# RedhawkSDR/psk_soft

Measured on AMD Instinct MI355X. Metric: complex IQ Msamples/s, QPSK 8 sps, 4096 ch; % HBM roofline at 1/2/4/8 GPUs, higher is better.
Workload: dtype f32

## Files before the change

### psk_soft_amd/csrc/psk_capi.cpp

```cpp
#include <hip/hip_runtime_api.h>
#include <hip/hip_vector_types.h>

#include <atomic>
#include <cmath>
#include <condition_variable>
#include <cstdio>
#include <cstdlib>
#include <cstring>
#include <functional>
#include <mutex>
#include <new>
#include <string>
#include <thread>
#include <vector>

#include "psk_acquire.h"
#include "psk_ctl.h"
#include "psk_gather.h"
#include "psk_plan.h"
#include "psk_quality.h"
#include "psk_soft_hip.h"
#include "psk_tune.h"

namespace psk {
// ... 600 lines not shown
    const psk::ChanCtl &c0 = h->ctl[ch0];
    for (uint32_t i = 1; i < nch; i++)
        if (!ctl_equal(c0, h->ctl[ch0 + i])) {
            h->mixed_lo = ch0, h->mixed_hi = ch0 + nch, h->mixed_ttl = 256;
            return nullptr;
        }
    psk_soft_handle::UniRun *run = nullptr;
    for (int k = psk_soft_handle::kUniRuns - 1; k >= 0; k--)
        run = h->uni[k].hi == h->uni[k].lo ? &h->uni[k] : run;
    if (!run) {
        run = &h->uni[0];
        run_sync(h, *run);
    }
    run->lo = ch0, run->hi = ch0 + nch, run->lazy = false;
    return run;
}
void plan_stamped(Round &r)
{
    psk_soft_handle *const h = r.h;
    if (!h->opt_stamp || r.cont || r.nch < 16u || !(r.run = uniform_run(h, r.ch0, r.nch)))
        return;
    r.stamp_ctl = r.run->lazy ? r.run->ctl : h->ctl[r.ch0];
    psk::ChanPlan &p0 = r.plans[0];
    const psk_soft_packet_t &k0 = r.pkts[0];
    if (psk::plan_call(r.stamp_ctl, r.lim, k0, r.outs[0], p0, false) != PSK_SOFT_OK || p0.mode == psk::PLAN_SKIP || misaligned(r, p0))
        return;
    p0.lf_flags |= r.extra_flags;
    p0.handed_over = r.handed_over;
    account(p0, r.lim, r.res, r.nch);
    const psk_soft_output_t o0 = r.outs[0];
    uint32_t i = 1;
    for (const uint32_t n = r.res.long_call ? 0u : r.nch; i < n; i++) {
        const psk_soft_packet_t &k = r.pkts[i];
        psk_soft_output_t &o = r.outs[i];
        if (k.n_floats != k0.n_floats || k.format != k0.format || k.present != k0.present || k.sri_mode != k0.sri_mode || k.sriChanged != k0.sriChanged ||
            k.inputQueueFlushed != k0.inputQueueFlushed || std::memcmp(&k.sri_xdelta, &k0.sri_xdelta, sizeof(double)) != 0)
            break;
        if (p0.n_out > o.cap_symbols && (o.soft || o.phase))
            break;
        psk::ChanPlan &p = r.plans[i];
        p = p0;
        p.in = k.data, p.soft = o.soft, p.bits = o.bits, p.phase = o.phase, p.sidx = o.sampleIndex;
        if (misaligned(r, p))
            break;
        o.ret = o0.ret, o.n_symbols = o0.n_symbols, o.n_bits = o0.n_bits, o.n_sampleIndex = o0.n_sampleIndex;
        o.sri_pushed = o0.sri_pushed, o.sri_soft_xdelta = o0.sri_soft_xdelta, o.sri_bits_xdelta = o0.sri_bits_xdelta;
        o.n_warn = o0.n_warn;
    }
    r.stamped = i == r.nch;
    if (!r.stamped)
        r.res = PlanSummary();
}
void plan_each(Round &r)
{
    psk::ChanCtl *const next = r.h->ctl_next.data() + r.ch0;
    const psk::ChanCtl *const cur = r.h->ctl.data() + r.ch0;
    PlanSummary &res = r.res;
    for (uint32_t i = 0; i < r.nch; i++) {
        next[i] = cur[i];
        psk::ChanPlan &p = r.plans[i];
        psk_soft_status st = psk::plan_call(next[i], r.lim, r.pkts[i], r.outs[i], p, r.cont && (r.cont[i] & 1u));
        if (st != PSK_SOFT_OK) {
            res.st = st, res.bad = i, res.why = st == PSK_SOFT_ERR_INVALID_ARG ? 3 : 0;
            return;
        }
        if (p.mode == psk::PLAN_SKIP)
            continue;
        if (misaligned(r, p)) {
            res.st = PSK_SOFT_ERR_INVALID_ARG, res.bad = i, res.why = 2;
            return;
        }
        p.lf_flags |= r.extra_flags;
        p.handed_over = r.handed_over;
        if (r.cont && (r.cont[i] & 2u))
            p.lf_flags |= psk::PLAN_NO_WRAP;
        if (r.cont && (r.cont[i] & 4u))
            p.lf_flags |= psk::PLAN_CARRY_DRIFT;
        account(p, r.lim, res, 1u);
    }
}
psk_soft_status refusal(const Round &r)
{
    const PlanSummary &res = r.res;
    if (res.why == 2)
        return fail(PSK_SOFT_ERR_INVALID_ARG,
                    "psk_soft_process: packet data must be 8-byte aligned (CS16: 4) (CS8: 2) (CF16: 4), soft 8, bits 4, phase 4, sampleIndex 4");
    char buf[160];
    if (res.why == 3) {
        std::snprintf(buf, sizeof buf, "psk_soft_process: channel %u: unknown packet format %u (PSK_SOFT_FORMAT_CF32 = 0, CS16 = 1, CS8 = 3, CF16 = 4)",
                      r.ch0 + res.bad, (unsigned)r.pkts[res.bad].format);
        return fail(PSK_SOFT_ERR_INVALID_ARG, buf);
    }
    std::snprintf(buf, sizeof buf, "psk_soft_process: channel %u refused (status %d)", r.ch0 + res.bad, (int)res.st);
    return fail(res.st, buf);
}
void commit(Round &r)
{
    psk_soft_handle *const h = r.h;
    if (r.stamped) {
        r.run->ctl = r.stamp_ctl;
        r.run->mode = r.plans[0].mode;
        r.run->lazy = true;
        return;
    }
    if (r.ch0 == 0 && r.nch == h->nch)
        h->ctl.swap(h->ctl_next);
    else
        std::memcpy(static_cast<void *>(h->ctl.data() + r.ch0), h->ctl_next.data() + r.ch0, sizeof(psk::ChanCtl) * r.nch);
    for (uint32_t i = 0; i < r.nch; i++) h->last_mode[r.ch0 + i] = r.plans[i].mode;
}
psk_soft_status wait_for_overlapping_calls(Round &r)
{
    psk_soft_handle *const h = r.h;
    for (int k = 0; k < kPlanSlots; k++)
        if (k != r.slot && h->ev_used[k] && h->slot_stream[k] != r.stream && h->slot_ch0[k] < r.ch0 + r.nch &&
            r.ch0 < h->slot_ch0[k] + h->slot_nch[k]) {
            PSK_HIP(hipStreamWaitEvent(r.stream, h->ev[k], 0));
            for (int a = 0; a < kAuxStreams; a++)
                if (h->slot_aux_used[k][a])
                    PSK_HIP(hipStreamWaitEvent(r.stream, h->slot_aux_ev[k][a], 0));
        }
    return PSK_SOFT_OK;
}
void move_in_place_back(Round &r)
{
    const psk_soft_handle *const h = r.h;
    if (r.stamped && !(r.plans[0].lf_flags & kInPlaceFlags))
        return;
    for (int S = 2; S <= 16; S++) {
        LaunchSet &fl = r.res.cls[S][1];
        uint32_t cnt = fl.cnt, mb = fl.max_blocks, mn = fl.max_n;
        for (const psk::PktFormat &f : psk::kPktFormats) {
            const LaunchSet &c = r.res.cls[S][f.cls];
            cnt += c.cnt;
            mb = c.max_blocks > mb ? c.max_blocks : mb;
            mn = c.max_n > mn ? c.max_n : mn;
        }
        if (cnt == fl.cnt || !h->opt_tiled || !psk::tile_front_has(S, 1))
            continue;
        const bool pipe = h->opt_pipe == 2 ? mb >= 4u
                                           : h->opt_pipe && h->opt_tiled == 1 && cnt >= kPipeMinChannels && cnt <= kPipeMaxChannels &&
                                                 mb >= kPipeMinBlocks && !r.cont && mn + 128u <= kPipeMaxYLen;
        const bool tiled = h->opt_tiled == 2 || pipe || (cnt <= kTiledFewChannels && mb >= kTiledMinBlocksFew) ||
                           (cnt <= kTiledMaxChannels && mb >= kTiledMinBlocks);
        if (!tiled)
            continue;
        fl.cnt = cnt, fl.max_blocks = mb, fl.max_n = mn;
        for (const psk::PktFormat &f : psk::kPktFormats) {
            LaunchSet &c = r.res.cls[S][f.cls];
            fl.max_A = fl.max_A > c.max_A ? fl.max_A : c.max_A;
            fl.blocks += c.blocks;
            c = LaunchSet{};
        }
        for (uint32_t i = 0; i < r.nch; i++)
            if (r.plans[i].S == (uint32_t)S)
                r.plans[i].lf_flags &= ~kInPlaceFlags;
    }
}
void fill_lists(Round &r)
{
    r.h_list = reinterpret_cast<uint32_t *>(r.h->h_plans[r.slot] + r.nch);
    r.d_plans = r.h->d_plans[r.slot];
    r.d_list = reinterpret_cast<const uint32_t *>(r.d_plans + r.nch);
    uint32_t run = 0;
    each_set(r.res, [&](LaunchSet &s) {
        s.off = run;
        run += s.cnt;
    });
    r.far_rows = r.res.anyf.cnt + r.res.widef.cnt + r.res.quietf.cnt;
    if (r.stamped) {
        for (uint32_t i = 0; i < r.nch; i++) r.h_list[i] = i;
        return;
    }
    for (uint32_t i = 0; i < r.nch; i++)
        if (LaunchSet *const s = set_of(r.plans[i], r.lim, r.res))
            r.h_list[s->off++] = i;
    each_set(r.res, [](LaunchSet &s) { s.off -= s.cnt; });
}
struct TileRule {
    uint64_t k_min;
    uint32_t z;
    bool lengthen;
    bool pfit;
};
void place_tiles(Round &r, LaunchSet &s, const TileRule &rule)
{
    const uint64_t blocks_z = s.blocks * rule.z;
    uint64_t K = blocks_z / kTiledTargetTiles;
    K = K < rule.k_min ? rule.k_min : K > 16 ? 16 : K;
    const uint64_t k_win = (s.max_A + 127u) / 128u;
    if (rule.lengthen && K < k_win) {
        const uint64_t k_fill = blocks_z / (kTiledTargetTiles / 2);
        const uint64_t k_long = k_win > 64 ? 64 : k_win;
        K = k_fill > k_long ? k_long : k_fill > K ? k_fill : K;
    }
    s.tiled = true;
    s.K = (uint8_t)K;
    s.tiles_max = (uint32_t)((s.max_blocks + K - 1) / K);
    for (uint32_t i = 0; i < s.cnt; i++) {
        psk::ChanPlan &p = r.plans[r.h_list[s.off + i]];
        const uint64_t nb = (p.n_out + 127u) / 128u;
        p.lf_flags |= psk::PLAN_TILED;
        if (rule.pfit && r.h->opt_pfit && p.lf_len0 == p.lf_n && p.lf_n >= 2)
            p.lf_flags |= psk::PLAN_PFIT;
        p.tile_blocks = (uint32_t)K;
        p.tile_base = (uint32_t)r.tile_count;
        p.tile_off = r.tile_syms;
        r.tile_count += (size_t)((nb + K - 1) / K);
        r.tile_syms += (size_t)nb * 128u;
    }
}
void place_ranges(Round &r, LaunchSet &s)
{
    s.piped = true;
    const uint32_t T = s.tiles_max;
    uint32_t tr = (uint32_t)(kTiledTargetTiles / s.cnt);
    tr = tr < 1u ? 1u : tr;
    if (r.h->opt_pipe == 2 && tr > 3u)
        tr = 3u;
    if (const char *e = std::getenv("PSK_SOFT_PIPE_RANGE_TILES"))
        tr = std::atoi(e) > 0 ? (uint32_t)std::atoi(e) : tr;
    if ((T + tr - 1) / tr > kPipeMaxRanges)
        tr = (T + kPipeMaxRanges - 1) / kPipeMaxRanges;
    s.pipe_tiles = tr;
    if (s.off + s.cnt > r.pipe_need)
        r.pipe_need = s.off + s.cnt;
}
void place_all(Round &r)
{
    const psk_soft_handle *const h = r.h;
    PlanSummary &res = r.res;
    r.wide_z = (res.wide.cnt || res.widef.cnt) ? psk::wide_chunks(res.wide.max_S > res.widef.max_S ? res.wide.max_S : res.widef.max_S) : 0u;
    if (res.wide.cnt)
        place_tiles(r, res.wide, TileRule{1, r.wide_z, true, true});
    if (res.widef.cnt)
        place_tiles(r, res.widef, TileRule{1, r.wide_z, true, false});
    r.wide_rec_need = r.tile_syms * r.wide_z * psk::wide_rec_bytes(), r.wide_stat_need = r.tile_count * r.wide_z * psk::wide_stat_bytes();
    if (res.any.cnt)
        place_tiles(r, res.any, TileRule{2, 1, true, true});
    if (res.anyf.cnt)
        place_tiles(r, res.anyf, TileRule{2, 1, true, false});
    r.pf_syms = r.tile_syms, r.pf_count = r.tile_count;
    for (int pass = 0; pass < (h->opt_tiled ? 2 : 0); pass++) {
        for (int S : kFastS)
            for (int H : kClassH) {
                LaunchSet &s = res.cls[S][H];
                if (!s.cnt || class_pkt(H) || !psk::tile_front_has(S, class_H(H)))
                    continue;
                const bool pipe = (h->opt_pipe == 2 ? s.max_blocks >= 4u
                                                    : h->opt_pipe && h->opt_tiled == 1 && s.cnt >= kPipeMinChannels && s.cnt <= kPipeMaxChannels &&
                                                          s.max_blocks >= kPipeMinBlocks) &&
                                  !r.cont && s.max_n + 128u <= kPipeMaxYLen && (size_t)s.blocks * 128u <= kPipeMaxSymbols;
                if (pipe != (pass == 1))
                    continue;
                if (!pipe && h->opt_tiled == 1 &&
                    !((s.cnt <= kTiledFewChannels && s.max_blocks >= kTiledMinBlocksFew) || (s.cnt <= kTiledMaxChannels && s.max_blocks >= kTiledMinBlocks)))
                    continue;
                place_tiles(r, s, TileRule{2, 1, false, !pipe});
                if (pipe)
                    place_ranges(r, s);
            }
        if (pass == 0)
            r.pf_syms = r.tile_syms, r.pf_count = r.tile_count;
    }
}

struct ScratchBuf {
    void **buf;
    size_t bytes;
};
template <class T>
inline ScratchBuf scratch_buf(T **p, size_t n) { return ScratchBuf{reinterpret_cast<void **>(p), sizeof(T) * n}; }
inline size_t plus_quarter(size_t need) { return need + need / 4; }
hipError_t grow_scratch(std::initializer_list<ScratchBuf> bufs, bool *got)
{
    if (const hipError_t e = hipDeviceSynchronize())
        return e;
    for (const ScratchBuf &b : bufs) (void)hipFree(*b.buf), *b.buf = nullptr;
    *got = true;
    for (const ScratchBuf &b : bufs) *got = *got && hipMalloc(b.buf, b.bytes) == hipSuccess;
    if (!*got) {
        (void)hipGetLastError();
        for (const ScratchBuf &b : bufs) (void)hipFree(*b.buf), *b.buf = nullptr;
    }
    return hipSuccess;
}
void to_reference_order(psk::ChanPlan &p)
{
    p.mode = p.S == 1u ? psk::PLAN_SEQ_S1 : psk::PLAN_SEQ;
    p.lf_flags &= ~(uint32_t)(psk::PLAN_TILED | psk::PLAN_PFIT | psk::PLAN_ANYFRONT | psk::PLAN_FARFIT);
}
psk_soft_status scratch_tiles(Round &r)
{
    psk_soft_handle *const h = r.h;
    PlanSummary &res = r.res;
    if (!r.tile_syms || (r.tile_syms <= h->tile_sym_cap && r.tile_count <= h->tile_cap && r.pf_syms <= h->pf_sym_cap && r.pf_count <= h->pf_cap))
        return PSK_SOFT_OK;
    h->tile_cap = h->tile_sym_cap = h->pf_cap = h->pf_sym_cap = 0;
    const size_t syms = plus_quarter(r.tile_syms), cnt = plus_quarter(r.tile_count);
    const size_t psyms = plus_quarter(r.pf_syms) + 128u, pcnt = plus_quarter(r.pf_count) + 1u;
    psk::PfScratch &pf = h->pf;
    bool got = false;
    PSK_HIP(grow_scratch({scratch_buf(&h->d_tiles, cnt), scratch_buf(&h->d_traw, syms), scratch_buf(&h->d_test, syms), scratch_buf(&h->d_ts, syms),
                          scratch_buf(&pf.k, psyms), scratch_buf(&pf.y, psyms), scratch_buf(&pf.S, psyms), scratch_buf(&pf.c, psyms),
                          scratch_buf(&pf.tt, psyms), scratch_buf(&pf.xs, psyms), scratch_buf(&pf.tile, pcnt),
                          scratch_buf(&pf.blk, psyms / 128u + 1u), scratch_buf(&pf.walk, psyms / 128u + 1u)},
                         &got));
    if (got && !pf.chan) {
        got = hipMalloc((void **)&pf.chan, sizeof(psk::PfChan) * h->nch) == hipSuccess &&
              hipMemset(pf.chan, 0, sizeof(psk::PfChan) * h->nch) == hipSuccess && hipHostMalloc((void **)&pf.hint, 64) == hipSuccess;
        if (got)
            *pf.hint = 0u;
    }
    if (got) {
        h->tile_cap = cnt, h->tile_sym_cap = syms, h->pf_cap = pcnt, h->pf_sym_cap = psyms;
        return PSK_SOFT_OK;
    }
    (void)hipGetLastError();
    for (uint32_t i = 0; i < r.nch; i++) {
        psk::ChanPlan &p = r.plans[i];
        if (p.lf_flags & psk::PLAN_ANYFRONT) {
            to_reference_order(p);
            res.any_seq = true;
        }
        p.lf_flags &= ~(uint32_t)(psk::PLAN_TILED | psk::PLAN_PFIT);
    }
    res.any.cnt = res.wide.cnt = res.anyf.cnt = res.widef.cnt = 0;
    for (int S : kFastS)
        for (int H : kClassH) res.cls[S][H].tiled = res.cls[S][H].piped = false;
    r.tile_syms = 0;
    return PSK_SOFT_OK;
}
psk_soft_status scratch_wide(Round &r)
{
    psk_soft_handle *const h = r.h;
    PlanSummary &res = r.res;
    if (!(res.wide.cnt || res.widef.cnt) || (r.wide_rec_need <= h->wide_rec_cap && r.wide_stat_need <= h->wide_stat_cap))
        return PSK_SOFT_OK;
    h->wide_rec_cap = h->wide_stat_cap = 0;
    const size_t rb = plus_quarter(r.wide_rec_need), sb = plus_quarter(r.wide_stat_need);
    bool got = false;
    PSK_HIP(grow_scratch({ScratchBuf{&h->d_wide_rec, rb}, ScratchBuf{&h->d_wide_stat, sb}}, &got));
    if (got) {
        h->wide_rec_cap = rb, h->wide_stat_cap = sb;
        return PSK_SOFT_OK;
    }
    for (const LaunchSet *s : {&res.wide, &res.widef})
        for (uint32_t i = 0; i < s->cnt; i++) to_reference_order(r.plans[r.h_list[s->off + i]]);
    res.wide.cnt = res.widef.cnt = 0;
    res.any_seq = true;
    return PSK_SOFT_OK;
}
psk_soft_status scratch_far_rows(Round &r)
{
    psk_soft_handle *const h = r.h;
    PlanSummary &res = r.res;
    if (!r.far_rows)
        return PSK_SOFT_OK;
    const uint32_t *const list = r.h_list + res.anyf.off;
    if (h->far_row.empty())
        h->far_row.assign(h->nch, 0u);
    uint32_t used = h->far_rows_used;
    for (uint32_t i = 0; i < r.far_rows; i++)
        if (!h->far_row[r.ch0 + list[i]])
            used++;
    bool got = true;
    if (used > h->far_rows_cap) {
        h->far_rows_cap = 0;
        const uint32_t cap = plus_quarter(used) < h->nch ? (uint32_t)plus_quarter(used) : h->nch;
        PSK_HIP(grow_scratch({ScratchBuf{(void **)&h->d_far_y, psk::far_ring_bytes() * cap}}, &got));
        if (got)
            h->far_rows_cap = cap;
    }
    for (uint32_t i = 0; i < r.far_rows; i++) {
        psk::ChanPlan &p = r.plans[list[i]];
        if (got) {
            uint32_t &row = h->far_row[r.ch0 + list[i]];
            if (!row)
                row = ++h->far_rows_used;
            p.far_row = row - 1u;
        } else if (p.n_out) {
            to_reference_order(p);
        }
    }
    if (!got) {
        if (res.quietf.cnt)
            return fail(PSK_SOFT_ERR_HIP, "psk_soft_process: out of device memory for the fit window of a far channel (PSK_SOFT_OPT_FAR_FIT)");
        res.anyf.cnt = res.widef.cnt = 0;
        res.any_seq = true;
    }
    return PSK_SOFT_OK;
}
psk_soft_status scratch_wide_seq(Round &r)
{
    psk_soft_handle *const h = r.h;
    for (uint32_t i = 0; i < r.nch; i++)
        if (r.plans[i].mode != psk::PLAN_SKIP && r.plans[i].S > kSeqMaxS) {
            r.n_wide_seq++;
            r.wide_seq_S = r.plans[i].S > r.wide_seq_S ? r.plans[i].S : r.wide_seq_S;
        }
    const size_t need = (size_t)r.n_wide_seq * r.wide_seq_S;
    if (need <= h->wide_symE_cap)
        return PSK_SOFT_OK;
    h->wide_symE_cap = 0;
    bool got = false;
    PSK_HIP(grow_scratch({scratch_buf(&h->d_wide_symE, plus_quarter(need))}, &got));
    if (!got)
        return fail(PSK_SOFT_ERR_HIP, "psk_soft_process: out of device memory for the symbolEnergy rows of wide symbols");
    h->wide_symE_cap = plus_quarter(need);
    return PSK_SOFT_OK;
}
psk_soft_status scratch_order(Round &r)
{
    psk_soft_handle *const h = r.h;
    if (!r.tile_syms && !r.n_wide_seq)
        return PSK_SOFT_OK;
    if (!h->tile_ev)
        PSK_HIP(hipEventCreateWithFlags(&h->tile_ev, hipEventDisableTiming));
    if (r.tile_syms) {
        if (h->pf.hint && *static_cast<volatile uint32_t *>(h->pf.hint)) {
            *static_cast<volatile uint32_t *>(h->pf.hint) = 0u;
            h->pf_second_ttl = 16;
        } else if (h->pf_second_ttl) {
            h->pf_second_ttl--;
        }
        r.pf_second = h->opt_pfit == 2 || h->pf_second_ttl > 0;
    }
    if (h->tile_ev_used && h->tile_stream != r.stream)
        PSK_HIP(hipStreamWaitEvent(r.stream, h->tile_ev, 0));
    if (!r.tile_syms || !r.pipe_need)
        return PSK_SOFT_OK;
    if (r.pipe_need > h->pipe_cap) {
        h->pipe_cap = 0;
        const size_t cap = plus_quarter(r.pipe_need);
        bool got = false;
        PSK_HIP(grow_scratch({ScratchBuf{&h->d_pipe_carry, psk::pipe_carry_bytes() * cap}, scratch_buf(&h->d_pipe_y, kPipeMaxYLen * cap)}, &got));
        if (got)
            h->pipe_cap = cap;
        else
            for (int S : kFastS)
                for (int H : kClassH) r.res.cls[S][H].piped = false;
    }
    if (!h->pipe_st[0]) {
        int prio_lo = 0, prio_hi = 0;
        PSK_HIP(hipDeviceGetStreamPriorityRange(&prio_lo, &prio_hi));
        for (hipStream_t &q : h->pipe_st) PSK_HIP(hipStreamCreateWithPriority(&q, hipStreamNonBlocking, prio_hi));
        for (hipEvent_t &e : h->pipe_ev) PSK_HIP(hipEventCreateWithFlags(&e, hipEventDisableTiming));
    }
    return PSK_SOFT_OK;
}
int cvt_format(const psk::ChanPlan &p)
{
    if (p.mode == psk::PLAN_SKIP || !p.n_in)
        return -1;
    for (int f = 0; f < psk::kNumPktFormats; f++)
        if ((p.lf_flags & psk::kPktFormats[f].flag) && !(p.lf_flags & psk::kPktFormats[f].in_place))
            return f;
    return -1;
}
psk_soft_status conversion_descriptors(Round &r)
{
    psk_soft_handle *const h = r.h;
    size_t need = 0;
    for (uint32_t i = 0; i < r.nch; i++)
        if (const int f = cvt_format(r.plans[i]); f >= 0) {
            need += align_up(sizeof(float2) * r.plans[i].n_in, 128);
            r.n_cvt++, r.n_cvt_f[f]++;
        }
    if (!r.n_cvt)
        return PSK_SOFT_OK;
    CvtScratch *cv = &h->cvt[0], *own = nullptr;
    for (auto &c : h->cvt) {
        cv = c.last_use < cv->last_use ? &c : cv;
        own = !own && c.buf && c.stream == r.stream ? &c : own;
    }
    r.cv = cv = own ? own : cv;
    if (!cv->ev)
        PSK_HIP(hipEventCreateWithFlags(&cv->ev, hipEventDisableTiming));
    if (cv->ev_used && cv->stream != r.stream)
        PSK_HIP(hipStreamWaitEvent(r.stream, cv->ev, 0));
    if (need > cv->cap) {
        cv->cap = 0;
        const size_t cap = align_up(plus_quarter(need), 4096);
        bool got = false;
        PSK_HIP(grow_scratch({ScratchBuf{(void **)&cv->buf, cap}}, &got));
        if (!got)
            return fail(PSK_SOFT_ERR_HIP, "psk_soft_process: out of device memory for the conversion of CS16 / CS8 / CF16 packets");
        cv->cap = cap;
    }
    cv->stream = r.stream, cv->last_use = ++h->cvt_calls;
    psk::CvtDesc *const desc =
        reinterpret_cast<psk::CvtDesc *>(reinterpret_cast<char *>(psk::plan_header(h->h_plans[r.slot])) + slot_cvt_offset(r.nch));
    size_t off = 0;
    uint32_t next[psk::kNumPktFormats] = {};
    for (int f = 1; f < psk::kNumPktFormats; f++) next[f] = next[f - 1] + r.n_cvt_f[f - 1];
    for (uint32_t i = 0; i < r.nch; i++) {
        psk::ChanPlan &p = r.plans[i];
        const int f = cvt_format(p);
        if (f < 0)
            continue;
        const uint32_t k = next[f]++;
        desc[k].src = reinterpret_cast<const uint32_t *>(p.in);
        desc[k].dst = reinterpret_cast<float *>(reinterpret_cast<char *>(cv->buf) + off);
        desc[k].n = p.n_in;
        p.in = desc[k].dst;
        off += align_up(sizeof(float2) * p.n_in, 128);
        r.cvt_max_n[f] = p.n_in > r.cvt_max_n[f] ? p.n_in : r.cvt_max_n[f];
    }
    return PSK_SOFT_OK;
}
void reference_order_lists(Round &r)
{
    for (uint32_t i = 0; i < r.nch; i++)
        for (int f = 0; f < psk::kNumPktFormats; f++) r.n_in_place_f[f] += (r.plans[i].lf_flags & psk::kPktFormats[f].in_place) ? 1u : 0u;
    for (const uint32_t n : r.n_in_place_f) r.n_in_place += n;
    r.n_seq_narrow = r.nch - r.n_in_place - r.n_wide_seq;
    if (!r.n_in_place && !r.n_wide_seq)
        return;
    uint32_t *const seq = reinterpret_cast<uint32_t *>(reinterpret_cast<char *>(psk::plan_header(r.h->h_plans[r.slot])) + slot_seq_offset(r.nch));
    uint32_t a = 0, b[psk::kNumPktFormats] = {r.n_seq_narrow}, c = r.nch - r.n_wide_seq;
    for (int f = 1; f < psk::kNumPktFormats; f++) b[f] = b[f - 1] + r.n_in_place_f[f - 1];
    for (uint32_t i = 0; i < r.nch; i++) {
        uint32_t *at = &a;
        for (int f = 0; f < psk::kNumPktFormats; f++)
            if (r.plans[i].lf_flags & psk::kPktFormats[f].in_place)
                at = &b[f];
        if (r.plans[i].mode != psk::PLAN_SKIP && r.plans[i].S > kSeqMaxS)
            at = &c;
        seq[(*at)++] = i;
    }
}
const char *invalid_plan(const Round &r, const psk::ChanPlan &p)
{
    const psk_soft_handle *const h = r.h;
    const uint64_t S = p.S ? p.S : 1u, have = (uint64_t)p.ring_len0 + p.n_in;
    const uint64_t nb = (p.n_out + 127u) / 128u;
    const bool emits = p.mode == psk::PLAN_FAST && p.n_out;
    const uint64_t tiles_end = p.tile_blocks ? (uint64_t)p.tile_base + (nb + p.tile_blocks - 1u) / p.tile_blocks : 0u;
    if (p.n_out && p.S > 1u && (p.n_out + p.A - 1u) * S > have)
        return "the call reads samples behind the packet's end";
    if (p.n_out && p.S <= 1u && p.mode != psk::PLAN_SEQ_S1 && p.n_out > p.n_in)
        return "more symbols than samples at one sample per symbol";
    if (p.ring_len0 > h->lim.ring_cap || p.ring_len1 > h->lim.ring_cap || p.ring_src > 1u)
        return "carried samples beyond the ring";
    if (p.ring_len1 > have)
        return "more samples carried out of the call than it holds";
    if (p.lf_n >= h->lim.fit_cap || p.lf_len0 > p.lf_n || p.lf_head >= h->lim.fit_cap)
        return "LinearFit window beyond its ring";
    if ((p.lf_flags & psk::PLAN_TILED) && emits && (!p.tile_blocks || p.tile_off + nb * 128u > h->tile_sym_cap || tiles_end > h->tile_cap))
        return "place in the time-tiled scratch outside it";
    if ((p.lf_flags & psk::PLAN_FARFIT) && emits &&
        (!h->d_far_y || p.far_row >= h->far_rows_cap || (p.lf_flags & psk::PLAN_PFIT) || p.lf_n < 128u))
        return "far fit without a row of its scratch";
    if ((p.lf_flags & psk::PLAN_PFIT) && emits && (p.tile_off + nb * 128u > h->pf_sym_cap || tiles_end > h->pf_cap))
        return "place in the parallel fit's scratch outside it";
    if (emits && !(p.lf_flags & psk::PLAN_ANYFRONT) && (p.S < 2u || p.S > 32u || p.A > 1024u || (p.S > 16u && p.A > 512u)))
        return "window class without a wave-scan instantiation planned for one";
    if (p.mode == psk::PLAN_FAST && p.n_out > psk::kResyncCount)
        return "a piece longer than 2^20 symbols on the wave-scan kernels";
    if ((p.lf_flags & psk::PLAN_TILED) && (p.lf_flags & psk::PLAN_ANYFRONT) && p.S > kSeqMaxS && emits &&
        (psk::wide_chunks(p.S) > r.wide_z || (p.tile_off + nb * 128u) * r.wide_z * psk::wide_rec_bytes() > h->wide_rec_cap ||
         tiles_end * r.wide_z * psk::wide_stat_bytes() > h->wide_stat_cap))
        return "place in the wide-symbol scratch outside it";
    if (p.S > kSeqMaxS && (p.S > r.wide_seq_S || !h->d_wide_symE || (size_t)r.n_wide_seq * r.wide_seq_S > h->wide_symE_cap))
        return "wide symbol without a row of symbolEnergy";
    if (cvt_format(p) >= 0 && (!r.cv || (const char *)p.in < (const char *)r.cv->buf ||
                               (const char *)p.in + sizeof(float2) * p.n_in > (const char *)r.cv->buf + r.cv->cap))
        return "converted CS16 / CS8 / CF16 packet outside the conversion scratch";
    return nullptr;
}
psk_soft_status validate(const Round &r)
{
    for (uint32_t i = 0; i < r.nch; i++)
        if (const char *const why = r.plans[i].mode == psk::PLAN_SKIP ? nullptr : invalid_plan(r, r.plans[i])) {
            char buf[200];
            std::snprintf(buf, sizeof buf, "psk_soft_process: plan of channel %u fails validation: %s", r.ch0 + i, why);
            return fail(PSK_SOFT_ERR_LIMIT, buf);
        }
    return PSK_SOFT_OK;
}
psk_soft_status choose_schedule(Round &r, bool *cut)
{
    psk_soft_handle *const h = r.h;
    const PlanSummary &res = r.res;
    for (int k = kNumClassH - 1; k >= 0; k--)
        for (int S : kFastS)
            if (res.cls[S][kClassH[k]].cnt)
                r.cls[r.n_cls++] = Cls{S, kClassH[k]};
    r.fork = r.n_cls > 1 && h->opt_fork;
    uint32_t listed = res.quiet.cnt, longest = 0;
    for (int i = 0; i < r.n_cls; i++) {
        const LaunchSet &s = res.cls[r.cls[i].S][r.cls[i].H];
        listed += s.cnt;
        longest = s.max_blocks > longest ? s.max_blocks : longest;
    }
    const bool wave_scan_only = r.fork && !r.tile_syms && !res.any.cnt && !res.any_seq && !r.n_cvt && !r.n_wide_seq;
    r.deferred = wave_scan_only && (h->opt_deferred || g_split_mode) && (!r.cont || g_split_mode);
    if (wave_scan_only && !r.cont && !h->opt_deferred && h->opt_split > 1) {
        static const uint32_t min_blocks = [] {
            const char *e = std::getenv("PSK_SOFT_SPLIT_MIN_BLOCKS");
            return e && std::atoi(e) > 0 ? (uint32_t)std::atoi(e) : kSplitMinBlocks;
        }();
        if (listed == r.nch && longest >= min_blocks) {
            *cut = true;
            return PSK_SOFT_OK;
        }
    }
    r.sig = 1469598103934665603ull;
// ... 213 lines not shown
        PSK_HIP(psk::launch_seq(r.d_plans, nullptr, r.ch0, r.nch, h->d_state, h->d_ring, h->lim.ring_cap, h->d_yv, h->lim.fit_cap, st));
        return PSK_SOFT_OK;
    }
    const uint32_t *const d_seq =
        reinterpret_cast<const uint32_t *>(reinterpret_cast<const char *>(psk::plan_header(r.d_plans)) + slot_seq_offset(r.nch));
    PSK_HIP(psk::launch_seq(r.d_plans, d_seq, r.ch0, r.n_seq_narrow, h->d_state, h->d_ring, h->lim.ring_cap, h->d_yv, h->lim.fit_cap, st));
    const uint32_t *d_seq_f = d_seq + r.n_seq_narrow;
    for (int f = 0; f < psk::kNumPktFormats; d_seq_f += r.n_in_place_f[f], f++)
        PSK_HIP(psk::launch_seq_pkt((int)psk::kPktFormats[f].id, r.d_plans, d_seq_f, r.ch0, r.n_in_place_f[f], h->d_state, h->d_ring, h->lim.ring_cap,
                                    h->d_yv, h->lim.fit_cap, st));
    if (r.n_wide_seq)
        PSK_HIP(mark(r, st, "seq_wide (reference order, samplesPerBaud > 1024)", (int)r.wide_seq_S, 0, ~0u, 0, 0, 0, 0));
    PSK_HIP(psk::launch_seq_wide(r.d_plans, d_seq + (r.nch - r.n_wide_seq), r.ch0, r.n_wide_seq, h->d_state, h->d_ring, h->lim.ring_cap, h->d_yv,
                                 h->lim.fit_cap, h->d_wide_symE, r.wide_seq_S, st));
    return PSK_SOFT_OK;
}
psk_soft_status enqueue(Round &r)
{
    psk_soft_handle *const h = r.h;
    const PlanSummary &res = r.res;
    const hipStream_t stream = r.stream;
    const psk::CvtDesc *d_desc = reinterpret_cast<const psk::CvtDesc *>(reinterpret_cast<const char *>(psk::plan_header(r.d_plans)) + slot_cvt_offset(r.nch));
    for (int f = 0; f < psk::kNumPktFormats; d_desc += r.n_cvt_f[f], f++) {
        if (!r.n_cvt_f[f])
            continue;
        PSK_HIP(mark(r, stream, psk::kPktFormats[f].convert, 0, 0, ~0u, 0, r.n_cvt_f[f], 0, 0));
        PSK_HIP(psk::launch_convert((int)psk::kPktFormats[f].id, d_desc, r.n_cvt_f[f], r.cvt_max_n[f], stream));
    }
    if (res.quiet.cnt) {
        const uint32_t y_len = ring_floats(res.quiet.max_n, 512u);
        PSK_HIP(mark(r, stream, "fast<0,1> (calls that emit nothing)", 0, 1, res.quiet.off, res.quiet.cnt, 0, y_len, 0));
        PSK_HIP(psk::launch_fast(0, 1, 0, r.d_plans, r.d_list + res.quiet.off, r.ch0, res.quiet.cnt, h->d_state, h->d_ring, h->lim.ring_cap, h->d_yv,
                                 h->lim.fit_cap, y_len, 0u, stream));
    }
    PSK_TRY(enqueue_any_sets(r));
    if (res.quiet.cnt && r.deferred)
        PSK_HIP(psk::launch_seq(r.d_plans, r.d_list + res.quiet.off, r.ch0, res.quiet.cnt, h->d_state, h->d_ring, h->lim.ring_cap, h->d_yv,
                                h->lim.fit_cap, stream));
    if (r.fork) {
        if (!h->aux_fork) {
            PSK_HIP(hipEventCreateWithFlags(&h->aux_fork, hipEventDisableTiming));
            int prio_lo = 0, prio_hi = 0;
            PSK_HIP(hipDeviceGetStreamPriorityRange(&prio_lo, &prio_hi));
            for (int k = 0; k < kAuxStreams; k++) {
                const char *pe = getenv("PSK_SOFT_AUX_PRIO");
                const int mode = pe ? atoi(pe) : 1;
                if (mode == 0 || prio_lo == prio_hi)
                    PSK_HIP(hipStreamCreateWithFlags(&h->aux[k], hipStreamNonBlocking));
                else
                    PSK_HIP(hipStreamCreateWithPriority(&h->aux[k], hipStreamNonBlocking, mode == 1 ? prio_hi : prio_lo));
                PSK_HIP(hipEventCreateWithFlags(&h->aux_join[k], hipEventDisableTiming));
            }
        }
        PSK_HIP(hipEventRecord(h->aux_fork, stream));
    }
    int used_aux = 0;
    for (int i = 0; i < r.n_cls; i++) {
        hipStream_t st = stream;
        if (r.fork && i > 0) {
            const int a = (i - 1) % kAuxStreams;
            st = h->aux[a];
            if (i - 1 < kAuxStreams) {
                PSK_HIP(hipStreamWaitEvent(st, h->aux_fork, 0));
                used_aux = i;
            }
        }
        PSK_TRY(enqueue_class(r, r.cls[i].S, r.cls[i].H, st));
    }
    PSK_TRY(enqueue_join_and_tail(r, used_aux));
    if (r.tile_syms || r.n_wide_seq)
        PSK_HIP(hipEventRecord(h->tile_ev, stream));
    if (r.n_cvt) {
        PSK_HIP(hipEventRecord(r.cv->ev, stream));
        r.cv->ev_used = true;
    }
    PSK_HIP(hipEventRecord(h->ev[r.slot], stream));
    return PSK_SOFT_OK;
}
psk_soft_status process_round(psk_soft_handle_t *h, uint32_t ch0, uint32_t nch, const psk_soft_packet_t *pkts, psk_soft_output_t *outs,
                              void *stream_v, const uint8_t *cont)
{
    if (!h || !pkts || !outs || !nch || (uint64_t)ch0 + nch > h->nch)
        return fail(PSK_SOFT_ERR_INVALID_ARG, "psk_soft_process: bad arguments");
    if (h->poisoned)
        return fail(PSK_SOFT_ERR_HIP, "psk_soft_process: an earlier call failed inside HIP after its kernels were enqueued; the "
                                      "channel states are undefined -- destroy the handle (or import saved states into a new one)");
    Round r{h, ch0, nch, pkts, outs, cont, stream_v ? (hipStream_t)stream_v : h->stream, h->slot, h->dry,
            (h->opt_qpsk_sign_map ? (uint32_t)psk::PLAN_QPSK_SIGN_MAP : 0u) | (h->opt_ties_in_place ? 0u : (uint32_t)psk::PLAN_TIES_HANDOVER), h->lim};
    PSK_TRY(take_slot(r));
    plan_stamped(r);
    if (!r.stamped) {
        ctl_touch_range(h, ch0, ch0 + nch);
        plan_each(r);
    }
    if (r.res.st == PSK_SOFT_OK && r.res.long_call && !cont) {
        g_long_call = true;
        return PSK_SOFT_OK;
    }
    if (r.res.st != PSK_SOFT_OK)
        return refusal(r);
    if (h->dry || !r.res.any_plan) {
        commit(r);
        return PSK_SOFT_OK;
    }
    PSK_TRY(wait_for_overlapping_calls(r));
    move_in_place_back(r);
    fill_lists(r);
    place_all(r);
    for (psk_soft_status (*phase)(Round &) : {scratch_tiles, scratch_wide, scratch_far_rows, scratch_wide_seq, scratch_order, conversion_descriptors})
        PSK_TRY(phase(r));
    reference_order_lists(r);
    if (h->opt_validate)
        PSK_TRY(validate(r));
    bool cut = false;
    PSK_TRY(choose_schedule(r, &cut));
    if (cut) {
        g_split_pieces = h->opt_split;
        return PSK_SOFT_OK;
    }
    PSK_TRY(upload(r));
    const psk_soft_status est = enqueue(r);
    if (est != PSK_SOFT_OK) {
        h->poisoned = true;
        return est;
    }
    commit(r);
    if (r.tile_syms || r.n_wide_seq) {
        h->tile_ev_used = true;
        h->tile_stream = r.stream;
    }
    h->slot = (h->slot + 1) % kPlanSlots;
    h->ev_used[r.slot] = true;
    h->slot_stream[r.slot] = r.stream, h->slot_ch0[r.slot] = ch0, h->slot_nch[r.slot] = nch;
    return PSK_SOFT_OK;
}
#undef PSK_TRY
}

extern "C" {

uint32_t psk_soft_abi_version(void) { return PSK_SOFT_ABI_VERSION; }
const char *psk_soft_last_error(void) { return g_last_error.c_str(); }

psk_soft_status psk_soft_create(int device, uint32_t n_channels, const psk_soft_limits_t *limits,
                                psk_soft_handle_t **out)
{
    if (!out || !n_channels)
        return fail(PSK_SOFT_ERR_INVALID_ARG, "psk_soft_create: null output or zero channels");
    *out = nullptr;
    psk_soft_limits_t lim;
    lim.max_window_samples = 16384;
    lim.max_phase_avg = 512;
    lim.max_packet_complex = 1u << 20;
    if (limits)
        lim = *limits;
    if (lim.max_window_samples < 16 || lim.max_phase_avg < 1)
        return fail(PSK_SOFT_ERR_INVALID_ARG, "psk_soft_create: limits too small");
    psk_soft_handle *h = new (std::nothrow) psk_soft_handle();
    if (!h)
        return fail(PSK_SOFT_ERR_INVALID_ARG, "out of host memory");
    h->nch = n_channels;
    h->user = lim;
    h->lim.ring_cap = lim.max_window_samples;
    h->lim.fit_cap = lim.max_phase_avg + 1;
    h->lim.fast_fit_max = kFastFitMax;
    h->lim.force_seq = false;
    h->lim.far_fit = false;
    h->ctl.resize(n_channels);
    h->ctl_next.resize(n_channels);
    h->last_mode.assign(n_channels, psk::PLAN_SKIP);
    h->device = device;
    h->dry = (device == PSK_SOFT_DEVICE_NONE);
    if (h->dry) {
        h->quality_dry.assign(n_channels, psk_soft_quality_t{});
        h->acquire_dry.assign(n_channels, psk_soft_acquire_t{});
    }
    if (const char *e = std::getenv("PSK_SOFT_TIME_TILED"))
        h->opt_tiled = std::atoi(e) < 0 ? 0 : std::atoi(e) > 2 ? 2 : std::atoi(e);
    if (const char *e = std::getenv("PSK_SOFT_FAR_FIT"))
        h->opt_far_fit = std::atoi(e) != 0;
    h->lim.far_fit = h->opt_far_fit != 0;
    if (const char *e = std::getenv("PSK_SOFT_TIES_IN_PLACE"))
        h->opt_ties_in_place = std::atoi(e) != 0;
    if (const char *e = std::getenv("PSK_SOFT_TRACE_LAUNCHES"))
        h->opt_trace = std::atoi(e);
    if (const char *e = std::getenv("PSK_SOFT_VALIDATE"))
        h->opt_validate = std::atoi(e);
    if (const char *e = std::getenv("PSK_SOFT_DIAG_GATHER_ONLY"))
        h->opt_diag_gather_only = std::atoi(e) != 0;
    if (const char *e = std::getenv("PSK_SOFT_SPLIT_CLASSES"))
        h->opt_split = std::atoi(e) < 0 ? 0 : std::atoi(e) > 16 ? 16 : std::atoi(e);
    if (const char *e = std::getenv("PSK_SOFT_PIPELINED"))
        h->opt_pipe = std::atoi(e) < 0 ? 0 : std::atoi(e) > 2 ? 2 : std::atoi(e);
    if (const char *e = std::getenv("PSK_SOFT_DEFERRED_JOIN"))
        h->opt_deferred = std::atoi(e) != 0;
    if (const char *e = std::getenv("PSK_SOFT_STAMP"))
        h->opt_stamp = std::atoi(e) != 0;
    if (const char *e = std::getenv("PSK_SOFT_PARALLEL_FIT"))
        h->opt_pfit = std::atoi(e) < 0 ? 0 : std::atoi(e) > 2 ? 2 : std::atoi(e);
    if (!h->dry) {
        int ndev = 0;
        hipError_t e = hipGetDeviceCount(&ndev);
        if (e != hipSuccess || ndev <= 0 || device < 0 || device >= ndev) {
            delete h;
            return fail(PSK_SOFT_ERR_NO_DEVICE,
                        std::string("psk_soft_create: no usable HIP device (") +
                            (e != hipSuccess ? hipGetErrorString(e) : "device index out of range") + ")");
        }
        hipDeviceProp_t prop;
        if (hipSetDevice(device) != hipSuccess || hipGetDeviceProperties(&prop, device) != hipSuccess) {
            delete h;
            return fail(PSK_SOFT_ERR_NO_DEVICE, "psk_soft_create: hipSetDevice failed");
        }
        if (std::strncmp(prop.gcnArchName, "gfx950", 6) != 0) {
            delete h;
            return fail(PSK_SOFT_ERR_NO_DEVICE,
                        std::string("psk_soft_create: kernels are built for gfx950 only, device is ") + prop.gcnArchName);
        }
        auto bail = [&](const char *what, hipError_t e2) {
            std::string msg = std::string("psk_soft_create: ") + what + ": " + hipGetErrorString(e2);
            psk_soft_destroy(h);
            return fail(PSK_SOFT_ERR_HIP, msg);
        };
        hipError_t e2;
        if ((e2 = hipStreamCreateWithFlags(&h->stream, hipStreamNonBlocking)) != hipSuccess)
            return bail("hipStreamCreate", e2);
        size_t state_b = sizeof(psk::ChanState) * (size_t)n_channels;
        size_t ring_b = sizeof(float2) * 2u * (size_t)h->lim.ring_cap * n_channels;
        size_t yv_b = sizeof(float) * (size_t)h->lim.fit_cap * n_channels;
        if ((e2 = hipMalloc((void **)&h->d_state, state_b)) != hipSuccess) return bail("hipMalloc state", e2);
        if ((e2 = hipMalloc((void **)&h->d_ring, ring_b)) != hipSuccess) return bail("hipMalloc ring", e2);
        if ((e2 = hipMalloc((void **)&h->d_yv, yv_b)) != hipSuccess) return bail("hipMalloc yvals", e2);
        std::vector<psk::ChanState> init(n_channels);
        std::memset(init.data(), 0, state_b);
        for (auto &s : init) s.lf_den = 1.0f;
        if ((e2 = hipMemcpy(h->d_state, init.data(), state_b, hipMemcpyHostToDevice)) != hipSuccess)
            return bail("hipMemcpy state", e2);
        if ((e2 = hipMemset(h->d_ring, 0, ring_b)) != hipSuccess) return bail("hipMemset", e2);
        if ((e2 = hipMemset(h->d_yv, 0, yv_b)) != hipSuccess) return bail("hipMemset", e2);
        if ((e2 = hipMalloc((void **)&h->d_quality, sizeof(psk_soft_quality_t) * (size_t)n_channels)) != hipSuccess)
            return bail("hipMalloc quality", e2);
        if ((e2 = hipMemset(h->d_quality, 0, sizeof(psk_soft_quality_t) * (size_t)n_channels)) != hipSuccess) return bail("hipMemset", e2);
        if ((e2 = hipMalloc((void **)&h->d_acquire, sizeof(psk_soft_acquire_t) * (size_t)n_channels)) != hipSuccess)
            return bail("hipMalloc acquire", e2);
        if ((e2 = hipMemset(h->d_acquire, 0, sizeof(psk_soft_acquire_t) * (size_t)n_channels)) != hipSuccess) return bail("hipMemset", e2);
        for (int s = 0; s < kPlanSlots; s++) {
            char *hb = nullptr, *db = nullptr;
            if ((e2 = hipHostMalloc((void **)&hb, slot_bytes(n_channels))) != hipSuccess)
                return bail("hipHostMalloc plans", e2);
            std::memset(hb, 0, psk::kPlanHeaderBytes);
            h->h_plans[s] = reinterpret_cast<psk::ChanPlan *>(hb + psk::kPlanHeaderBytes);
            if ((e2 = hipMalloc((void **)&db, slot_bytes(n_channels))) != hipSuccess)
                return bail("hipMalloc plans", e2);
            h->d_plans[s] = reinterpret_cast<psk::ChanPlan *>(db + psk::kPlanHeaderBytes);
            if ((e2 = hipEventCreateWithFlags(&h->ev[s], hipEventDisableTiming)) != hipSuccess)
                return bail("hipEventCreate", e2);
            if ((e2 = hipEventCreateWithFlags(&h->ev_up[s], hipEventDisableTiming)) != hipSuccess)
                return bail("hipEventCreate", e2);
        }
        if ((e2 = hipStreamCreateWithFlags(&h->up_stream, hipStreamNonBlocking)) != hipSuccess)
            return bail("hipStreamCreate", e2);
        if (const char *e = std::getenv("PSK_SOFT_PLAN_STREAM"))
            h->opt_up_stream = std::atoi(e) != 0;
    }
    *out = h;
    return PSK_SOFT_OK;
}

psk_soft_status psk_soft_destroy(psk_soft_handle_t *h)
{
    if (!h)
        return PSK_SOFT_OK;
    if (!h->dry) {
        (void)hipSetDevice(h->device);
        if (h->stream)
            (void)hipStreamSynchronize(h->stream);
        for (int s = 0; s < kPlanSlots; s++) {
            if (h->h_plans[s]) (void)hipHostFree(psk::plan_header(h->h_plans[s]));
            if (h->d_plans[s]) (void)hipFree(psk::plan_header(h->d_plans[s]));
            if (h->ev[s]) (void)hipEventDestroy(h->ev[s]);
            if (h->ev_up[s]) (void)hipEventDestroy(h->ev_up[s]);
        }
        if (h->d_state) (void)hipFree(h->d_state);
        if (h->d_ring) (void)hipFree(h->d_ring);
        if (h->d_yv) (void)hipFree(h->d_yv);
        for (auto &q : h->qslot) {
            if (q.ev) (void)hipEventSynchronize(q.ev), (void)hipEventDestroy(q.ev);
            if (q.h_desc) (void)hipHostFree(q.h_desc);
            if (q.d_desc) (void)hipFree(q.d_desc);
            if (q.d_part) (void)hipFree(q.d_part);
        }
        if (h->d_quality) (void)hipFree(h->d_quality);
        for (auto &q : h->aslot) {
            if (q.ev) (void)hipEventSynchronize(q.ev), (void)hipEventDestroy(q.ev);
            if (q.h_desc) (void)hipHostFree(q.h_desc);
            if (q.d_desc) (void)hipFree(q.d_desc);
            if (q.d_part) (void)hipFree(q.d_part);
        }
        if (h->d_acquire) (void)hipFree(h->d_acquire);
        if (h->d_tiles) (void)hipFree(h->d_tiles);
        if (h->d_traw) (void)hipFree(h->d_traw);
        if (h->d_test) (void)hipFree(h->d_test);
        if (h->d_ts) (void)hipFree(h->d_ts);
        for (void *q : {(void *)h->pf.k, (void *)h->pf.y, (void *)h->pf.S, (void *)h->pf.c, (void *)h->pf.tt, (void *)h->pf.xs,
                        (void *)h->pf.tile, (void *)h->pf.blk, (void *)h->pf.walk, (void *)h->pf.chan})
            if (q) (void)hipFree(q);
        if (h->pf.hint) (void)hipHostFree(h->pf.hint);
        if (h->tile_ev) (void)hipEventDestroy(h->tile_ev);
        for (auto &cv : h->cvt) {
            if (cv.ev) (void)hipEventSynchronize(cv.ev), (void)hipEventDestroy(cv.ev);
            if (cv.buf) (void)hipFree(cv.buf);
        }
        for (auto &g : h->gat) {
            if (g.ev) (void)hipEventSynchronize(g.ev), (void)hipEventDestroy(g.ev);
            if (g.buf) (void)hipFree(g.buf);
        }
        for (auto &g : h->gdesc) {
            if (g.ev) (void)hipEventSynchronize(g.ev), (void)hipEventDestroy(g.ev);
            if (g.h_buf) (void)hipHostFree(g.h_buf);
            if (g.d_buf) (void)hipFree(g.d_buf);
        }
        if (h->d_tune_tab) (void)hipFree(h->d_tune_tab);
        for (auto &sl : h->stage) {
            if (sl.stream) (void)hipStreamSynchronize(sl.stream);
            if (sl.h_buf) (void)hipHostFree(sl.h_buf);
            if (sl.d_buf) (void)hipFree(sl.d_buf);
            if (sl.done) (void)hipEventDestroy(sl.done);
            if (sl.stream) (void)hipStreamDestroy(sl.stream);
        }
        delete h->pool;
        for (int k = 0; k < kAuxStreams; k++) {
            if (h->aux[k]) (void)hipStreamSynchronize(h->aux[k]);
            if (h->aux_join[k]) (void)hipEventDestroy(h->aux_join[k]);
            if (h->aux[k]) (void)hipStreamDestroy(h->aux[k]);
        }
        for (hipStream_t &q : h->pipe_st)
            if (q) {
                (void)hipStreamSynchronize(q);
                (void)hipStreamDestroy(q);
            }
        for (hipEvent_t &e : h->pipe_ev)
            if (e) (void)hipEventDestroy(e);
        if (h->d_pipe_carry) (void)hipFree(h->d_pipe_carry);
        if (h->d_pipe_y) (void)hipFree(h->d_pipe_y);
        if (h->d_wide_rec) (void)hipFree(h->d_wide_rec);
        if (h->d_wide_stat) (void)hipFree(h->d_wide_stat);
        if (h->d_wide_symE) (void)hipFree(h->d_wide_symE);
        if (h->d_far_y) (void)hipFree(h->d_far_y);
        if (h->aux_fork) (void)hipEventDestroy(h->aux_fork);
        for (auto &row : h->slot_aux_ev)
            for (hipEvent_t &e : row)
                if (e) (void)hipEventDestroy(e);
        if (h->up_stream) {
            (void)hipStreamSynchronize(h->up_stream);
            (void)hipStreamDestroy(h->up_stream);
        }
        if (h->stream) (void)hipStreamDestroy(h->stream);
    }
    delete h;
    return PSK_SOFT_OK;
}

psk_soft_status psk_soft_configure(psk_soft_handle_t *h, uint32_t ch0, uint32_t nch, const psk_soft_props_t *props)
{
    if (!h || !props || (uint64_t)ch0 + nch > h->nch)
        return fail(PSK_SOFT_ERR_INVALID_ARG, "psk_soft_configure: bad channel range");
    for (uint32_t i = 0; i < nch; i++) {
        const psk_soft_props_t &p = props[i];
        if ((uint64_t)p.samplesPerBaud * p.numAvg > h->lim.ring_cap || p.phaseAvg >= h->lim.fit_cap)
            return fail(PSK_SOFT_ERR_LIMIT, "psk_soft_configure: property exceeds the limits given at create "
                                            "(samplesPerBaud*numAvg, phaseAvg)");
    }
    ctl_touch(h);
    for (uint32_t i = 0; i < nch; i++) h->ctl[ch0 + i].configure(props[i]);
    return PSK_SOFT_OK;
}

psk_soft_status psk_soft_query(const psk_soft_handle_t *h, uint32_t ch, psk_soft_props_t *props)
{
    if (!h || !props || ch >= h->nch)
        return fail(PSK_SOFT_ERR_INVALID_ARG, "psk_soft_query: bad channel");
    ctl_sync(h);
    *props = h->ctl[ch].props;
    return PSK_SOFT_OK;
}

psk_soft_status psk_soft_fire_listener(psk_soft_handle_t *h, uint32_t ch, int which)
{
    if (!h || ch >= h->nch)
        return fail(PSK_SOFT_ERR_INVALID_ARG, "psk_soft_fire_listener: bad channel");
    ctl_touch(h);
    switch (which) {
    case 0: h->ctl[ch].samplesPerBaudChanged(); break;
    case 1: h->ctl[ch].constelationSizeChanged(); break;
    case 2: h->ctl[ch].phaseAvgChanged(); break;
    default: return fail(PSK_SOFT_ERR_INVALID_ARG, "psk_soft_fire_listener: which must be 0..2");
    }
    return PSK_SOFT_OK;
}

uint64_t psk_soft_output_capacity(const psk_soft_handle_t *h, uint32_t ch, uint64_t n_complex)
{
    if (!h || ch >= h->nch)
        return 0;
    ctl_sync(h);
    uint64_t S = h->ctl[ch].props.samplesPerBaud ? h->ctl[ch].props.samplesPerBaud : 1;
    return (n_complex + S - 1) / S + 1;
}

static psk_soft_status process_device_call(psk_soft_handle_t *h, uint32_t ch0, uint32_t nch, const psk_soft_packet_t *pkts,
                                           psk_soft_output_t *outs, void *stream_v)
{
    g_long_call = false;
    g_split_pieces = 0;
    {
        const psk_soft_status st = process_round(h, ch0, nch, pkts, outs, stream_v, nullptr);
        if (st != PSK_SOFT_OK || (!g_long_call && g_split_pieces < 2))
            return st;
        g_long_call = false;
    }
    const uint64_t split = g_split_pieces > 1 ? (uint64_t)g_split_pieces : 0;
    g_split_pieces = 0;
    struct SplitScope {
        bool on;
        explicit SplitScope(bool v) : on(v) { g_split_mode = v; }
        ~SplitScope() { g_split_mode = false; }
    } split_scope(split != 0);
    std::vector<uint64_t> piece_cap(split ? nch : 0, ~0ull);

    ctl_sync(h);
    std::vector<psk_soft_packet_t> pk(pkts, pkts + nch);
    std::vector<psk_soft_output_t> ou(outs, outs + nch), total(outs, outs + nch);
    std::vector<uint64_t> left(nch);
    std::vector<uint8_t> cont(nch, 0);
    std::vector<uint32_t> mode_of(nch, psk::PLAN_SKIP);
    for (uint32_t i = 0; i < nch; i++) left[i] = pkts[i].present ? pkts[i].n_floats : 0;
    for (int round = 0;; round++) {
        bool more = false;
        for (uint32_t i = 0; i < nch; i++) {
            psk_soft_packet_t &q = pk[i];
            if (round > 0) {
                q.present = left[i] ? 1 : 0;
                q.sriChanged = 0;
                q.inputQueueFlushed = 0;
            }
            cont[i] = round > 0 ? (split ? 5 : 1) : 0;
            if (!q.present || q.sri_mode != 1) {
                left[i] = 0;
                continue;
            }
            const psk::ChanCtl &c = h->ctl[ch0 + i];
            const uint64_t S = c.props.samplesPerBaud ? c.props.samplesPerBaud : 1, A = c.props.numAvg;
            uint64_t n_fl = left[i];
            for (int attempt = 0; attempt < 4; attempt++) {
                psk::ChanCtl probe = c;
                psk::ChanPlan pl;
                psk_soft_packet_t qq = q;
                qq.n_floats = n_fl;
                psk_soft_output_t oo = ou[i];
                oo.cap_symbols = ~0ull;
                if (psk::plan_call(probe, h->lim, qq, oo, pl, (cont[i] & 1u) != 0) != PSK_SOFT_OK)
                    break;
                uint64_t lim_sym = psk::kResyncCount - pl.lf_count0 < psk::kResyncCount ? psk::kResyncCount - pl.lf_count0 : psk::kResyncCount;
                if (split) {
                    if (round == 0 && attempt == 0)
                        piece_cap[i] = ((oo.n_symbols + split - 1) / split + 127ull) & ~127ull;
                    lim_sym = piece_cap[i] < lim_sym ? piece_cap[i] : lim_sym;
                }
                const bool last = n_fl == left[i];
                if (oo.n_symbols <= lim_sym && (last || (oo.n_symbols & 1ull) == 0))
                    break;
                uint64_t want = oo.n_symbols > lim_sym ? lim_sym : oo.n_symbols - 1;
                want &= ~1ull;
                const uint64_t excess = oo.n_symbols - want;
                const uint64_t cut = 2ull * S * excess;
                n_fl = n_fl > cut ? n_fl - cut : 2ull * S * (A + 2);
                (void)A;
            }
            if (n_fl < left[i])
                n_fl &= ~1ull;
            q.n_floats = n_fl;
            left[i] -= n_fl < left[i] ? n_fl : left[i];
            if (left[i])
                cont[i] |= 2u;
            more = more || left[i] != 0;
        }
        const psk_soft_status st = process_round(h, ch0, nch, pk.data(), ou.data(), stream_v, cont.data());
        if (st != PSK_SOFT_OK) {
            if (round > 0)
                h->poisoned = true;
            return st;
        }
        ctl_sync(h);
        for (uint32_t i = 0; i < nch; i++) {
            const psk_soft_output_t &o = ou[i];
            psk_soft_output_t &t = total[i];
            if (round == 0) {
                t = o;
                t.soft = outs[i].soft, t.bits = outs[i].bits, t.phase = outs[i].phase, t.sampleIndex = outs[i].sampleIndex;
                t.cap_symbols = outs[i].cap_symbols;
            } else if (pk[i].present) {
                t.n_symbols += o.n_symbols;
                t.n_bits += o.n_bits;
                t.n_sampleIndex += o.n_sampleIndex;
                t.n_warn += o.n_warn;
            }
            if (pk[i].present) {
                mode_of[i] = h->last_mode[ch0 + i];
                pk[i].data = pk[i].data ? reinterpret_cast<const float *>(reinterpret_cast<const char *>(pk[i].data) +
                                                                          elem_bytes(pk[i]) * pk[i].n_floats)
                                        : nullptr;
                pk[i].n_floats = left[i];
                if (ou[i].soft) ou[i].soft += 2 * o.n_symbols;
                if (ou[i].bits) ou[i].bits += o.n_bits;
                if (ou[i].phase) ou[i].phase += o.n_symbols;
                if (ou[i].sampleIndex) ou[i].sampleIndex += o.n_sampleIndex;
                ou[i].cap_symbols = ou[i].cap_symbols > o.n_symbols ? ou[i].cap_symbols - o.n_symbols : 0;
            }
        }
        if (!more)
            break;
    }
    ctl_sync(h);
    for (uint32_t i = 0; i < nch; i++) {
        outs[i] = total[i];
        h->last_mode[ch0 + i] = mode_of[i];
    }
    if (split && !h->dry && !h->opt_deferred) {
        PSK_HIP(hipSetDevice(h->device));
        PSK_HIP(deferred_join(h, stream_v ? (hipStream_t)stream_v : h->stream));
    }
    return PSK_SOFT_OK;
}

static psk_soft_status quality_pass(psk_soft_handle_t *h, uint32_t ch0, uint32_t nch, const psk_soft_output_t *outs, void *stream_v)
{
    const psk_soft_handle::QualitySnap *snap = h->q_snap.data();
    if (h->dry) {
        for (uint32_t i = 0; i < nch; i++) {
            psk_soft_quality_t r = {};
            r.n_symbols = outs[i].n_symbols;
            r.constelationSize = snap[i].M, r.samplesPerBaud = snap[i].S, r.differentialDecoding = snap[i].diff;
            r.flags = PSK_SOFT_Q_PLANNED;
            h->quality_dry[ch0 + i] = r;
        }
        return PSK_SOFT_OK;
    }
    PSK_HIP(hipSetDevice(h->device));
    hipStream_t stream = stream_v ? (hipStream_t)stream_v : h->stream;
    PSK_HIP(deferred_join(h, stream));
    QualitySlot &q = h->qslot[h->q_turn];
    if (q.used)
        PSK_HIP(hipEventSynchronize(q.ev));
    if (!q.ev)
        PSK_HIP(hipEventCreateWithFlags(&q.ev, hipEventDisableTiming));
    if (!q.h_desc)
        PSK_HIP(hipHostMalloc((void **)&q.h_desc, sizeof(psk::QualityDesc) * (size_t)h->nch));
    if (!q.d_desc)
        PSK_HIP(hipMalloc((void **)&q.d_desc, sizeof(psk::QualityDesc) * (size_t)h->nch));
    uint64_t n_seg = 0;
    uint32_t max_seg = 0;
    for (uint32_t i = 0; i < nch; i++) {
        const psk_soft_output_t &o = outs[i];
        psk::QualityDesc &d = q.h_desc[i];
        d = psk::QualityDesc{};
        d.channel = ch0 + i;
        d.M = snap[i].M, d.S = snap[i].S, d.diff = snap[i].diff;
        if (!o.n_symbols)
            continue;
        d.n_symbols = o.n_symbols;
        d.n_sidx = o.n_sampleIndex;
        uint32_t f = 0;
        if (o.soft)
            f |= PSK_SOFT_Q_SOFT | (d.M == 2 || d.M == 4 || d.M == 8 ? PSK_SOFT_Q_LOCK : 0);
        if (o.phase)
            f |= PSK_SOFT_Q_PHASE;
        if (o.sampleIndex && o.n_sampleIndex)
            f |= PSK_SOFT_Q_INDEX;
        d.flags = (uint8_t)f;
        d.soft = (f & PSK_SOFT_Q_SOFT) ? o.soft : nullptr;
        d.phase = (f & PSK_SOFT_Q_PHASE) ? o.phase : nullptr;
        d.sidx = (f & PSK_SOFT_Q_INDEX) ? o.sampleIndex : nullptr;
        if (f & (PSK_SOFT_Q_SOFT | PSK_SOFT_Q_INDEX)) {
            const uint64_t segs = (o.n_symbols + psk::kQualitySegSymbols - 1u) / psk::kQualitySegSymbols;
            if (n_seg + segs > 0x7fffffffull)
                return fail(PSK_SOFT_ERR_LIMIT, "psk_soft_process: too many symbols in one call for the quality pass");
            d.seg0 = (uint32_t)n_seg;
            d.n_seg = (uint32_t)segs;
            n_seg += segs;
            max_seg = d.n_seg > max_seg ? d.n_seg : max_seg;
        }
    }
    if (n_seg > q.part_cap) {
        if (q.d_part) (void)hipFree(q.d_part);
        q.d_part = nullptr;
        q.part_cap = 0;
        const size_t cap = (size_t)n_seg + (size_t)n_seg / 4u + 256u;
        PSK_HIP(hipMalloc((void **)&q.d_part, sizeof(psk::QualityPartial) * cap));
        q.part_cap = cap;
    }
    for (const QualitySlot &k : h->qslot)
        if (&k != &q && k.used && k.stream != stream && k.ch0 < ch0 + nch && ch0 < k.ch0 + k.nch)
            PSK_HIP(hipStreamWaitEvent(stream, k.ev, 0));
    PSK_HIP(hipMemcpyAsync(q.d_desc, q.h_desc, sizeof(psk::QualityDesc) * (size_t)nch, hipMemcpyHostToDevice, stream));
    q.used = true, q.stream = stream, q.ch0 = ch0, q.nch = nch;
    auto mark = [&](const char *what) -> hipError_t {
        if (!h->opt_trace)
// ... 1221 lines not shown
```

### psk_soft_amd/csrc/psk_pfit.h

```cpp
#ifndef PSK_PFIT_H
#define PSK_PFIT_H

#include "psk_fast_kernel.h"

namespace psk {

constexpr uint32_t kPfFailYSum = 1u, kPfFailXySum = 2u, kPfFailUnwrap = 4u;

PSK_DEV bool pf_mine(const ChanPlan &p) { return p.mode == PLAN_FAST && (p.lf_flags & PLAN_PFIT) && p.n_out != 0; }
PSK_DEV bool pf_in_round(const ChanPlan &p, const PfScratch &sc, uint32_t bi, int round) { return pf_mine(p) && (round == 0 || sc.chan[bi].retry != 0u); }

struct PfGeo {
    int lane, n_out, n_blocks, c_begin, c_end, tile;
    uint64_t off;
    uint32_t tbase;
    uint32_t bbase;
};
PSK_DEV bool pf_geo(const ChanPlan &p, PfGeo &g)
{
    g.lane = threadIdx.x & 63;
    g.n_out = (int)p.n_out;
    g.n_blocks = (g.n_out + kB - 1) / kB;
    g.tile = (int)blockIdx.x;
    g.c_begin = g.tile * (int)p.tile_blocks;
    g.c_end = g.c_begin + (int)p.tile_blocks < g.n_blocks ? g.c_begin + (int)p.tile_blocks : g.n_blocks;
    g.off = p.tile_off;
    g.tbase = p.tile_base;
    g.bbase = (uint32_t)(p.tile_off / kB);
    return g.c_begin < g.n_blocks;
}
PSK_DEV float pf_z(const ChanPlan &p, const float *y_row, const float *yv, uint32_t fit_cap, int t)
{
    const int n = (int)p.lf_n;
    return t >= n ? y_row[t - n] : yv[(p.lf_head + (uint32_t)t) % fit_cap];
}

constexpr float kPfSteep = 0.12f;
__global__ __launch_bounds__(64) void pf_unwrap_kernel(const ChanPlan *__restrict__ plans, const uint32_t *__restrict__ list, uint32_t ch0,
                                                       const ChanState *__restrict__ states, const float *__restrict__ t_raw, PfScratch sc)
{
    const uint32_t bi = list[blockIdx.y];
    const ChanPlan &p = plans[bi];
    PfGeo g;
    if (!pf_mine(p) || !pf_geo(p, g))
        return;
    const float *raw_row = t_raw + g.off;
    int *k_row = sc.k + g.off;
    const float inv2pi = 0.15915494f, two_pi = 6.2831853f;
    const ChanState &st = states[ch0 + bi];
    const bool steep = !(__builtin_fabsf(st.lf_m) < kPfSteep);
    int run = 0;
    if (steep) {
        for (int c = g.c_begin; c < g.c_end; c++) {
            const int i0 = c * kB + 2 * g.lane;
            const float2 rw = *reinterpret_cast<const float2 *>(raw_row + i0);
            const float before = c ? raw_row[c * kB - 1] : rw.x;
            const float prev = wave_up1(rw.y, before);
            int j0 = (int)__builtin_rintf((prev - rw.x) * inv2pi);
            const int j1 = (int)__builtin_rintf((rw.x - rw.y) * inv2pi);
            if (i0 == 0)
                j0 = 0;
            const int incl = wave_scan_i32(j0 + j1);
            const int k0 = run + wave_up1(incl, 0) + j0;
            *reinterpret_cast<int2 *>(k_row + i0) = make_int2(k0, k0 + j1);
            run += __builtin_amdgcn_readlane(incl, 63);
        }
    } else {
        float a_last = st.phaseEstimate;
        if (g.c_begin > 0) {
            const int t = g.c_begin * kB - 16 + 2 * (g.lane & 7);
            const float2 rw = *reinterpret_cast<const float2 *>(raw_row + t);
            float ph[2] = {__cosf(rw.x) + __cosf(rw.y), __sinf(rw.x) + __sinf(rw.y)};
            wave_scan_f32_multi(ph);
            a_last = atan2f(read_lane(ph[1], 7), read_lane(ph[0], 7));
        }
        const int grp = g.lane >> 3;
        for (int c = g.c_begin; c < g.c_end; c++) {
            const int i0 = c * kB + 2 * g.lane;
            const float2 rw = *reinterpret_cast<const float2 *>(raw_row + i0);
            const bool v0 = i0 < g.n_out, v1 = i0 + 1 < g.n_out;
            float ph[2] = {(v0 ? __cosf(rw.x) : 0.0f) + (v1 ? __cosf(rw.y) : 0.0f), (v0 ? __sinf(rw.x) : 0.0f) + (v1 ? __sinf(rw.y) : 0.0f)};
            wave_scan_f32_multi(ph);
            const int hi = (g.lane | 7) << 2, lo = ((g.lane & ~7) - 1) << 2;
            const float re = bperm_addr(hi, ph[0]) - (grp ? bperm_addr(lo, ph[0]) : 0.0f);
            const float im = bperm_addr(hi, ph[1]) - (grp ? bperm_addr(lo, ph[1]) : 0.0f);
            const float a = atan2f(im, re);
            const float a_left = bperm_addr(lo, a);
            const float a_prev = grp ? a_left : a_last;
            const int jb = (g.lane & 7) == 0 ? (int)__builtin_rintf((a_prev - a) * inv2pi) : 0;
            const int K = run + wave_scan_i32(jb);
            const float U = a + two_pi * (float)(K - run);
            const float U_l = bperm_addr(((g.lane & ~7) - 8) << 2, U), U_r = bperm_addr(((g.lane & ~7) + 8) << 2, U);
            const float slope = grp == 0 ? (U_r - U) * (1.0f / 16.0f) : grp == 7 ? (U - U_l) * (1.0f / 16.0f) : (U_r - U_l) * (1.0f / 32.0f);
            const float dt0 = (float)(2 * (g.lane & 7)) - 7.5f;
            const float line0 = a + slope * dt0, line1 = line0 + slope;
            const int k0 = K + (int)__builtin_rintf((line0 - rw.x) * inv2pi), k1 = K + (int)__builtin_rintf((line1 - rw.y) * inv2pi);
            *reinterpret_cast<int2 *>(k_row + i0) = make_int2(k0, k1);
            run = __builtin_amdgcn_readlane(K, 63);
            a_last = read_lane(a, 63);
        }
    }
    if (g.lane == 0)
        sc.tile[g.tbase + g.tile].jsum = run;
}

__global__ __launch_bounds__(64) void pf_y_kernel(const ChanPlan *__restrict__ plans, const uint32_t *__restrict__ list, uint32_t ch0,
                                                  const ChanState *__restrict__ states, const float *__restrict__ t_raw, PfScratch sc, int round)
{
    const uint32_t bi = list[blockIdx.y];
    const ChanPlan &p = plans[bi];
    PfGeo g;
    if (!pf_in_round(p, sc, bi, round) || !pf_geo(p, g))
        return;
    const float *raw_row = t_raw + g.off;
    int *k_row = sc.k + g.off;
    float *y_row = sc.y + g.off;
    int koff = 0;
    if (round == 0) {
        for (int j = g.lane; j < g.tile; j += kWave) koff += sc.tile[g.tbase + j].jsum;
        koff = __builtin_amdgcn_readlane(wave_scan_i32(koff), 63);
        if (!(__builtin_fabsf(states[ch0 + bi].lf_m) < kPfSteep))
            koff += (int)unwrap_count(states[ch0 + bi].phaseEstimate, (double)raw_row[0]);
    }
    float2 rw_n = *reinterpret_cast<const float2 *>(raw_row + g.c_begin * kB + 2 * g.lane);
    int2 k_n = *reinterpret_cast<const int2 *>(k_row + g.c_begin * kB + 2 * g.lane);
    for (int c = g.c_begin; c < g.c_end; c++) {
        const int i0 = c * kB + 2 * g.lane;
        const float2 rw = rw_n;
        int2 k = k_n;
        if (c + 1 < g.c_end) {
            rw_n = *reinterpret_cast<const float2 *>(raw_row + i0 + kB);
            k_n = *reinterpret_cast<const int2 *>(k_row + i0 + kB);
        }
        k.x += koff;
        k.y += koff;
        *reinterpret_cast<int2 *>(k_row + i0) = k;
        const double two_pi = PSK_KD(kTwoPi, c);
        const float y0 = (float)((double)rw.x + (double)(long long)k.x * two_pi);
        const float y1 = (float)((double)rw.y + (double)(long long)k.y * two_pi);
        *reinterpret_cast<float2 *>(y_row + i0) = make_float2(y0, y1);
    }
}

__global__ __launch_bounds__(64) void pf_ydiff_kernel(const ChanPlan *__restrict__ plans, const uint32_t *__restrict__ list, uint32_t ch0,
                                                      const float *__restrict__ yvs, uint32_t fit_cap, PfScratch sc, int round)
{
    const uint32_t bi = list[blockIdx.y];
    const ChanPlan &p = plans[bi];
    PfGeo g;
    if (!pf_in_round(p, sc, bi, round) || !pf_geo(p, g))
        return;
    const float *y_row = sc.y + g.off;
    const float *yv = yvs + (size_t)(ch0 + bi) * fit_cap;
    double *S_row = sc.S + g.off;
    double run = 0.0, dlast = 0.0;
    const int j0 = g.c_begin * kB + 2 * g.lane;
    float2 y_n = *reinterpret_cast<const float2 *>(y_row + j0);
    float z0_n = pf_z(p, y_row, yv, fit_cap, j0), z1_n = pf_z(p, y_row, yv, fit_cap, j0 + 1);
    for (int c = g.c_begin; c < g.c_end; c++) {
        const int i0 = c * kB + 2 * g.lane;
        const float2 y = y_n;
        const float z0 = z0_n, z1 = z1_n;
        if (c + 1 < g.c_end) {
            y_n = *reinterpret_cast<const float2 *>(y_row + i0 + kB);
            z0_n = pf_z(p, y_row, yv, fit_cap, i0 + kB);
            z1_n = pf_z(p, y_row, yv, fit_cap, i0 + kB + 1);
        }
        const bool v0 = i0 < g.n_out, v1 = i0 + 1 < g.n_out;
        const double d0 = v0 ? (double)y.x - (double)z0 : 0.0;
        const double d1 = v1 ? (double)y.y - (double)z1 : 0.0;
        const double incl = wave_scan_f64(d0 + d1);
        const double a0 = (run + wave_up1(incl, 0.0)) + d0;
        *reinterpret_cast<double2 *>(S_row + i0) = make_double2(a0, a0 + d1);
        run += read_lane(incl, 63);
        const int rem = g.n_out - c * kB;
        const int last = (rem < kB ? rem : kB) - 1;
        dlast = read_lane((last & 1) ? a0 + d1 : a0, last >> 1);
    }
    if (g.lane == 0) {
        sc.tile[g.tbase + g.tile].dsum = run;
        sc.tile[g.tbase + g.tile].dlast = dlast;
    }
}

__global__ __launch_bounds__(64) void pf_ysum_kernel(const ChanPlan *__restrict__ plans, const uint32_t *__restrict__ list, uint32_t ch0,
                                                     const ChanState *__restrict__ states, const float *__restrict__ yvs, uint32_t fit_cap,
                                                     PfScratch sc, int round)
{
    const uint32_t bi = list[blockIdx.y];
    const ChanPlan &p = plans[bi];
    PfGeo g;
    if (!pf_in_round(p, sc, bi, round) || !pf_geo(p, g))
        return;
    const float *y_row = sc.y + g.off;
    const float *yv = yvs + (size_t)(ch0 + bi) * fit_cap;
    double *S_row = sc.S + g.off;
    double *c_row = sc.c + g.off;
    float *t_row = sc.tt + g.off;
    double soff = 0.0;
    for (int j = g.lane; j < g.tile; j += kWave) soff += sc.tile[g.tbase + j].dsum;
    soff = sc.chan[bi].ySum_c + wave_sum_f64(soff);
    bool bad = false;
    if (g.tile > 0) {
        double soff_b = 0.0;
        for (int j = g.lane; j < g.tile - 1; j += kWave) soff_b += sc.tile[g.tbase + j].dsum;
        soff_b = sc.chan[bi].ySum_c + wave_sum_f64(soff_b);
        bad = !same_bits(soff_b + sc.tile[g.tbase + g.tile - 1].dlast, soff);
    }
    const float xd = p.lf_xdelta;
    const float sizef = (float)(p.lf_n - 1u);
    double S_before = soff;
    double xrun = 0.0;
    const int j0 = g.c_begin * kB + 2 * g.lane;
    float2 y_n = *reinterpret_cast<const float2 *>(y_row + j0);
    double2 dl_n = *reinterpret_cast<const double2 *>(S_row + j0);
    float z0_n = pf_z(p, y_row, yv, fit_cap, j0), z1_n = pf_z(p, y_row, yv, fit_cap, j0 + 1);
    for (int c = g.c_begin; c < g.c_end; c++) {
        const int i0 = c * kB + 2 * g.lane;
        const bool v0 = i0 < g.n_out, v1 = i0 + 1 < g.n_out;
        const float2 y = y_n;
        const double2 dl = dl_n;
        const float z0f = z0_n, z1f = z1_n;
        if (c + 1 < g.c_end) {
            y_n = *reinterpret_cast<const float2 *>(y_row + i0 + kB);
            dl_n = *reinterpret_cast<const double2 *>(S_row + i0 + kB);
            z0_n = pf_z(p, y_row, yv, fit_cap, i0 + kB);
            z1_n = pf_z(p, y_row, yv, fit_cap, i0 + kB + 1);
        }
        const double S0 = soff + dl.x, S1 = soff + dl.y;
        const double z0 = v0 ? (double)z0f : 0.0, z1 = v1 ? (double)z1f : 0.0;
        const double Sp = wave_up1(S1, S_before);
        const double a0 = Sp - z0, a1 = S0 - z1;
        bad = bad || (v0 && !same_bits(a0 + (double)y.x, S0)) || (v1 && !same_bits(a1 + (double)y.y, S1));
        const double c0 = (double)xd * a0, c1 = (double)xd * a1;
        float t0 = y.x * sizef;
        t0 = t0 * xd;
        float t1 = y.y * sizef;
        t1 = t1 * xd;
        *reinterpret_cast<double2 *>(S_row + i0) = make_double2(S0, S1);
        *reinterpret_cast<double2 *>(c_row + i0) = make_double2(c0, c1);
        *reinterpret_cast<float2 *>(t_row + i0) = make_float2(t0, t1);
        const double bs = wave_sum_f64((v0 ? (double)t0 - c0 : 0.0) + (v1 ? (double)t1 - c1 : 0.0));
        if (g.lane == 0)
            sc.blk[g.bbase + c].bsum = bs;
        xrun += bs;
        const int rem = g.n_out - c * kB;
        const int last = (rem < kB ? rem : kB) - 1;
        S_before = read_lane((last & 1) ? S1 : S0, last >> 1);
    }
    if (g.lane == 0)
        sc.tile[g.tbase + g.tile].xsum = xrun;
    if (vote_any(bad) && g.lane == 0)
        atomicOr(&sc.chan[bi].fail, kPfFailYSum);
}

struct PfGrid {
    bool T[kR], V[kR], E[kR], dpos[kR];
    double inc[kR], ch[kR];
};
PSK_DEV void pf_classify(double inv_q, bool modeB, const double (&c)[kR], const double (&t)[kR], PfGrid &gr)
{
#pragma unroll
    for (int r = 0; r < kR; r++) {
        const double nc = c[r] * inv_q, nt = t[r] * inv_q;
        const double ch = __builtin_rint(nc);
        gr.ch[r] = ch;
        gr.inc[r] = nt - ch;
        if (!modeB) {
            const double d = nc - ch;
            gr.T[r] = __builtin_fabs(d) == 0.5;
            gr.dpos[r] = d > 0.0;
            gr.E[r] = false;
            gr.V[r] = odd_f64(gr.inc[r]);
        } else {
            gr.T[r] = odd_f64(gr.inc[r]);
            const bool hw = odd_f64((gr.T[r] ? gr.inc[r] - 1.0 : gr.inc[r]) * 0.5);
            gr.E[r] = hw;
            gr.V[r] = !gr.T[r] && hw;
            gr.dpos[r] = false;
        }
    }
}
PSK_DEV void pf_resolve(int lane, bool modeB, bool P_c, const PfGrid &gr, double &a0, double &a1)
{
    const bool Ac = gr.T[0] || gr.T[1];
    const bool Vc = gr.T[1] ? gr.V[1] : (gr.V[0] != gr.V[1]);
    const unsigned long long mA = vote_mask(Ac), mV = vote_mask(Vc);
    const bool G = (__builtin_amdgcn_mbcnt_hi((unsigned)(mV >> 32), __builtin_amdgcn_mbcnt_lo((unsigned)mV, 0u)) & 1u) != 0;
    const unsigned long long mF = vote_mask(Ac && G);
    const unsigned long long lt = lane ? (~0ull >> (64 - lane)) : 0ull;
    const unsigned long long X = mA & lt, Y = mF & lt;
    const bool P_in = (X ? (Y > (X >> 1)) : P_c) != G;
    const bool sel0 = P_in != gr.E[0];
    const bool P0 = gr.T[0] ? gr.V[0] : (P_in != gr.V[0]);
    const bool sel1 = P0 != gr.E[1];
    if (!modeB) {
        a0 = gr.inc[0] + ((gr.T[0] && sel0) ? (gr.dpos[0] ? -1.0 : 1.0) : 0.0);
        a1 = gr.inc[1] + ((gr.T[1] && sel1) ? (gr.dpos[1] ? -1.0 : 1.0) : 0.0);
    } else {
        a0 = gr.inc[0] + (gr.T[0] ? (sel0 ? 1.0 : -1.0) : 0.0);
        a1 = gr.inc[1] + (gr.T[1] ? (sel1 ? 1.0 : -1.0) : 0.0);
    }
}

__global__ __launch_bounds__(64) void pf_xblock_kernel(const ChanPlan *__restrict__ plans, const uint32_t *__restrict__ list, uint32_t ch0,
                                                       const ChanState *__restrict__ states, PfScratch sc, int round)
{
    const uint32_t bi = list[blockIdx.y];
    const ChanPlan &p = plans[bi];
    PfGeo g;
    if (!pf_in_round(p, sc, bi, round) || !pf_geo(p, g))
        return;
    const double *c_row = sc.c + g.off;
    const float *t_row = sc.tt + g.off;
    double s_pred = 0.0;
    for (int j = g.lane; j < g.tile; j += kWave) s_pred += sc.tile[g.tbase + j].xsum;
    s_pred = sc.chan[bi].xySum_c + wave_sum_f64(s_pred);
    int prev_scale = -1;
    if (g.c_begin > 0) {
        const double s_before = s_pred - sc.blk[g.bbase + g.c_begin - 1].bsum;
        const int eb_b = (__double2hiint(s_before - c_row[(g.c_begin - 1) * kB]) >> 20) & 0x7ff;
        if (eb_b >= 60 && eb_b <= 2040)
            prev_scale = 2 * eb_b + (!(__builtin_fabs(s_before) < pow2_biased(eb_b + 1)) ? 1 : 0);
    }
    for (int c = g.c_begin; c < g.c_end; c++) {
        const int i0 = c * kB + 2 * g.lane;
        const bool v0 = i0 < g.n_out, v1 = i0 + 1 < g.n_out;
        const double2 cv = *reinterpret_cast<const double2 *>(c_row + i0);
        const float2 tv = *reinterpret_cast<const float2 *>(t_row + i0);
        const double cc[kR] = {v0 ? cv.x : 0.0, v1 ? cv.y : 0.0};
        const double tt[kR] = {v0 ? (double)tv.x : 0.0, v1 ? (double)tv.y : 0.0};
        const double c_first = read_lane(cc[0], 0);
        const double r_first = s_pred - c_first;
        const int eb = (__double2hiint(r_first) >> 20) & 0x7ff;
        PfBlock rec;
        rec.bsum = sc.blk[g.bbase + c].bsum;
        rec.a = __builtin_inf();
        rec.b = -__builtin_inf();
        rec.kmul = rec.D0s = rec.D1s = 0.0;
        rec.flags = rec.pad = 0;
        int scale_id = -1;
        if (eb >= 60 && eb <= 2040) {
            const double inv_q = pow2_biased(2098 - eb);
            const bool modeB = !(__builtin_fabs(s_pred) < pow2_biased(eb + 1));
            const bool neg = s_pred < 0.0;
            PfGrid gr;
            pf_classify(inv_q, modeB, cc, tt, gr);
            double a0, a1, b0, b1;
            pf_resolve(g.lane, modeB, false, gr, a0, a1);
            pf_resolve(g.lane, modeB, true, gr, b0, b1);
            const double incl = wave_scan_f64(a0 + a1);
            const double D0 = read_lane(incl, 63), D1 = wave_sum_f64(b0 + b1);
            const double sg = neg ? -1.0 : 1.0;
            const double e_before = sg * wave_up1(incl, 0.0);
            const double e0 = e_before + sg * a0, e1 = e0 + sg * a1;
            const double w0 = e_before - sg * gr.ch[0], w1 = e0 - sg * gr.ch[1];
            const float kUp = 1.0000002f;
            const float big = 3.0e38f;
            const float e_hi = wave_max_f32(__builtin_fmaxf(__builtin_fmaxf((float)e0, (float)e1) * kUp, 0.0f));
            const float e_lo = wave_max_f32(__builtin_fmaxf(__builtin_fmaxf(-(float)e0, -(float)e1) * kUp, 0.0f));
            const float w0f = v0 ? (float)w0 : -big, w1f = v1 ? (float)w1 : -big;
            const float n0f = v0 ? -(float)w0 : -big, n1f = v1 ? -(float)w1 : -big;
            const float scale = wave_max_f32(__builtin_fmaxf(__builtin_fabsf(v0 ? (float)w0 : 0.0f), __builtin_fabsf(v1 ? (float)w1 : 0.0f))) * kUp + 1.0f;
            const float w_hi = wave_max_f32(__builtin_fmaxf(__builtin_fmaxf(w0f, w1f) + scale, 0.0f)) * kUp - scale * 0.999999f;
            const float w_lo = wave_max_f32(__builtin_fmaxf(__builtin_fmaxf(n0f, n1f) + scale, 0.0f)) * kUp - scale * 0.999999f;
            const double slack = 300.0;
            const double two52 = 4503599627370496.0, two53 = 9007199254740992.0;
            const double r_lo = two52 + (double)w_lo + slack, r_hi = two53 - (double)w_hi - slack;
            double lo, hi;
            if (!modeB) {
                lo = r_lo;
                const double s_hi = two53 - (double)e_hi - slack;
                hi = s_hi < r_hi ? s_hi : r_hi;
            } else {
                const double s_lo = two53 + (double)e_lo + slack;
                lo = s_lo > r_lo ? s_lo : r_lo;
                hi = r_hi;
            }
            if (lo < hi) {
                const double q = pow2_biased(eb - 52);
                rec.a = neg ? -(hi * q) : lo * q;
                rec.b = neg ? -(lo * q) : hi * q;
                rec.kmul = inv_q * (modeB ? 0.25 : 0.5);
                rec.D0s = D0 * q;
                rec.D1s = D1 * q;
                scale_id = 2 * eb + (modeB ? 1 : 0);
                const bool f0 = modeB ? odd_f64(D0 * 0.5) : odd_f64(D0), f1 = modeB ? odd_f64(D1 * 0.5) : odd_f64(D1);
                rec.flags = (f0 ? 1 : 0) | (f1 ? 2 : 0) | ((scale_id == prev_scale) ? 4 : 0);
            }
        }
        prev_scale = scale_id;
        if (g.lane == 0)
            sc.blk[g.bbase + c] = rec;
        s_pred += rec.bsum;
    }
}

PSK_DEV bool pf_x_ok(double s_c, const bool (&valid)[kR], const double (&c)[kR], const double (&t)[kR], const double (&xs)[kR])
{
    const double xp = wave_up1(xs[1], s_c);
    const bool x0 = same_bits((xp - c[0]) + t[0], xs[0]), x1 = same_bits((xs[0] - c[1]) + t[1], xs[1]);
    return vote_all((x0 || !valid[0]) && (x1 || !valid[1]));
}

struct PfOps {
    double2 cv;
    float2 tv;
};
PSK_DEV PfOps pf_load_ops(int lane, int b, const double *c_row, const float *t_row)
{
    const int i0 = b * kB + 2 * lane;
    PfOps o;
    o.cv = *reinterpret_cast<const double2 *>(c_row + i0);
    o.tv = *reinterpret_cast<const float2 *>(t_row + i0);
    return o;
}
PSK_DEV double pf_walk_block(int lane, int b, int n_out, double s_c, const PfOps &ops, double *xs_row, bool try_grid, bool &grid_failed)
{
    const int i0 = b * kB + 2 * lane;
    const bool valid[kR] = {i0 < n_out, i0 + 1 < n_out};
#ifdef PSK_DIAG_WALK_NOLOAD
    const double2 cv = make_double2(s_c * 0.25, s_c * 0.125);
    const float2 tv = make_float2((float)lane, 1.0f);
#else
    const double2 cv = ops.cv;
    const float2 tv = ops.tv;
#endif
    const double cc[kR] = {valid[0] ? cv.x : 0.0, valid[1] ? cv.y : 0.0};
    const double tt[kR] = {valid[0] ? (double)tv.x : 0.0, valid[1] ? (double)tv.y : 0.0};
    double xs[kR];
    bool done = false;
#ifdef PSK_DIAG_WALK_NOCHAIN
    xs[0] = s_c - cc[0], xs[1] = s_c - tt[1];
    done = true;
#endif
    if (try_grid && !done) {
        xysum_grid(lane, s_c, cc, tt, xs);
        done = pf_x_ok(s_c, valid, cc, tt, xs);
        grid_failed = !done;
    }
    if (!done) {
        double x = s_c;
#pragma unroll 1
        for (int k = 0; k < kWave; k += PSK_CHAIN_UNROLL) {
#pragma unroll
            for (int u = 0; u < PSK_CHAIN_UNROLL; u++) {
                const double bb = wave_up1(x, s_c);
                x = ((bb - cc[0]) + tt[0] - cc[1]) + tt[1];
            }
        }
        const double b_fin = wave_up1(x, s_c);
        xs[0] = (b_fin - cc[0]) + tt[0];
        xs[1] = x;
    }
    *reinterpret_cast<double2 *>(xs_row + i0) = make_double2(xs[0], xs[1]);
    const int rem = n_out - b * kB;
    const int last = (rem < kB ? rem : kB) - 1;
    return read_lane((last & 1) ? xs[1] : xs[0], last >> 1);
}

PSK_DEV double pf_from_lane(double v, int src)
{
    const int lo = bperm_addr(src << 2, __double2loint(v)), hi = bperm_addr(src << 2, __double2hiint(v));
    return __hiloint2double(hi, lo);
}
__global__ __launch_bounds__(64) void pf_xwalk_kernel(const ChanPlan *__restrict__ plans, const uint32_t *__restrict__ list,
                                                      const PfBlock *__restrict__ blk_all, PfScratch sc, int round)
{
    const uint32_t bi = list[blockIdx.x];
    const ChanPlan &p = plans[bi];
    if (!pf_in_round(p, sc, bi, round))
        return;
    const int lane = threadIdx.x & 63;
    const int n_out = (int)p.n_out;
    const int n_blocks = (n_out + kB - 1) / kB;
    const PfBlock *const blk = blk_all + (uint32_t)(p.tile_off / kB);
    PfWalk *const walk = sc.walk + (uint32_t)(p.tile_off / kB);
    const double *c_row = sc.c + p.tile_off;
    const float *t_row = sc.tt + p.tile_off;
    double *xs_row = sc.xs + p.tile_off;
    double s_c = sc.chan[bi].xySum_c;
    uint32_t slow_blocks = 0;
#ifdef PSK_DIAG_WALK_TIME
    const unsigned long long t_begin = wall_clock64();
#endif
    int par = -1;
    for (int b0 = 0; b0 < n_blocks; b0 += kWave) {
        const bool have = b0 + lane < n_blocks;
        const PfBlock rec = blk[have ? b0 + lane : n_blocks - 1];
        const int nb = n_blocks - b0 < kWave ? n_blocks - b0 : kWave;
        const bool usable = have && rec.a < rec.b;
        double s_in_mine = 0.0;
        int slow_mine = 0;
        int start = 0;
        while (start < nb) {
#ifdef PSK_DIAG_WALK_SCANS
            slow_blocks += 1000u;
#endif
            const int fl_s = __builtin_amdgcn_readlane(rec.flags, start);
            if (par < 0 || !(fl_s & 4))
                par = (__builtin_amdgcn_fract(s_c * read_lane(rec.kmul, start)) != 0.0) ? 1 : 0;
            par = __builtin_amdgcn_readfirstlane(par);
            const bool in_run = lane >= start && usable;
            double dS0 = in_run ? rec.D0s : 0.0, dS1 = in_run ? rec.D1s : 0.0;
            int out = in_run ? ((rec.flags & 1) ? 1 : 0) | ((rec.flags & 2) ? 0 : 2) : 2;
#pragma unroll
            for (int d = 1; d < kWave; d <<= 1) {
                const int src = lane - d;
                const bool take = src >= start;
                const double l0 = pf_from_lane(dS0, src), l1 = pf_from_lane(dS1, src);
                const int lout = bperm_addr(src << 2, out);
                if (take) {
                    const int o0 = lout & 1, o1 = (lout >> 1) & 1;
                    const double r0 = dS0, r1 = dS1;
                    dS0 = l0 + (o0 ? r1 : r0);
                    dS1 = l1 + (o1 ? r1 : r0);
                    out = ((out >> o0) & 1) | (((out >> o1) & 1) << 1);
                }
            }
            const double s_after = s_c + (par ? dS1 : dS0);
            const int par_after = (out >> par) & 1;
            const double s_left = pf_from_lane(s_after, lane - 1);
            const double s_before = lane > start ? s_left : s_c;
            const bool inside = lane >= start && lane < nb;
            const bool enter_ok = usable && rec.a < s_before && s_before < rec.b && (lane == start || (rec.flags & 4));
            const unsigned long long stops = vote_mask(inside && !enter_ok);
            const int f = stops ? (int)__builtin_ctzll(stops) : nb;
            if (lane >= start && lane < f)
                s_in_mine = s_before;
            if (f > start) {
                s_c = read_lane(s_after, f - 1);
                par = __builtin_amdgcn_readlane(par_after, f - 1);
            }
            if (f >= nb)
                break;
            const double a_f = read_lane(rec.a, f), b_f = read_lane(rec.b, f);
            if (a_f < s_c && s_c < b_f && f > start) {
                par = -1;
                start = f;
                continue;
            }
            int fs = f;
            PfOps ops = pf_load_ops(lane, b0 + fs, c_row, t_row);
            bool grid_first = !(a_f < b_f);
            bool grid_failed = false;
            for (;;) {
                const bool more = fs + 1 < nb;
                PfOps ahead = ops;
                if (more)
                    ahead = pf_load_ops(lane, b0 + fs + 1, c_row, t_row);
                if (lane == fs) {
                    s_in_mine = s_c;
                    slow_mine = 1;
                }
                s_c = pf_walk_block(lane, b0 + fs, n_out, s_c, ops, xs_row, grid_first, grid_failed);
                slow_blocks++;
                start = fs + 1;
                if (!more)
                    break;
                const double a_n = read_lane(rec.a, fs + 1), b_n = read_lane(rec.b, fs + 1);
                if (a_n < s_c && s_c < b_n)
                    break;
                fs++;
                ops = ahead;
                grid_first = !(a_n < b_n) && !grid_failed;
            }
            par = -1;
        }
        if (have) {
            PfWalk w;
            w.s_in = s_in_mine;
            w.slow = slow_mine;
            w.pad = 0;
            walk[b0 + lane] = w;
        }
    }
#ifdef PSK_DIAG_WALK_TIME
    slow_blocks = (uint32_t)((wall_clock64() - t_begin) / 1u);
#endif
    if (lane == 0)
        sc.chan[bi].slow_blocks = slow_blocks;
}

__global__ __launch_bounds__(64) void pf_verify_kernel(const ChanPlan *__restrict__ plans, const uint32_t *__restrict__ list, uint32_t ch0,
                                                       const ChanState *__restrict__ states, const float *__restrict__ yvs, uint32_t fit_cap,
                                                       const float *__restrict__ t_raw, float *__restrict__ t_est, PfScratch sc, int round)
{
    const uint32_t bi = list[blockIdx.y];
    const ChanPlan &p = plans[bi];
    PfGeo g;
    if (!pf_in_round(p, sc, bi, round) || !pf_geo(p, g))
        return;
    const ChanState &st = states[ch0 + bi];
    const float *raw_row = t_raw + g.off;
    const int *k_row = sc.k + g.off;
    const float *y_row = sc.y + g.off;
    const double *S_row = sc.S + g.off;
    const float *yv = yvs + (size_t)(ch0 + bi) * fit_cap;
    double *xs_row = sc.xs + g.off;
    float *est_row = t_est + g.off;
    const uint32_t n = p.lf_n;
    const float xd = p.lf_xdelta;
    const float sizef = (float)(p.lf_n - 1u);
    float den_s = st.lf_den, xavg_s = st.lf_xavg;
    fit_denominator(xd, n, den_s, xavg_s);
    const FitKnown fk = fit_known(xd, n, den_s, xavg_s);
    bool bad = false, bad_k = false;
    for (int c = g.c_begin; c < g.c_end; c++) {
        const int i0 = c * kB + 2 * g.lane;
        const bool valid[kR] = {i0 < g.n_out, i0 + 1 < g.n_out};
        const PfWalk *rec = sc.walk + g.bbase + c;
        const double s_c = rec->s_in;
        const double2 Sv = *reinterpret_cast<const double2 *>(S_row + i0);
        const float2 y = *reinterpret_cast<const float2 *>(y_row + i0);
        const double S_front = c ? S_row[c * kB - 1] : sc.chan[bi].ySum_c + 0.0;
        const double Sp = wave_up1(Sv.y, S_front);
        const double z0 = valid[0] ? (double)pf_z(p, y_row, yv, fit_cap, i0) : 0.0, z1 = valid[1] ? (double)pf_z(p, y_row, yv, fit_cap, i0 + 1) : 0.0;
        const double a0 = Sp - z0, a1 = Sv.x - z1;
        float t0 = y.x * sizef;
        t0 = t0 * xd;
        float t1 = y.y * sizef;
        t1 = t1 * xd;
        const double cc[kR] = {valid[0] ? (double)xd * a0 : 0.0, valid[1] ? (double)xd * a1 : 0.0};
        const double tt[kR] = {valid[0] ? (double)t0 : 0.0, valid[1] ? (double)t1 : 0.0};
        double xs[kR];
        if (rec->slow) {
            const double2 xv = *reinterpret_cast<const double2 *>(xs_row + i0);
            xs[0] = xv.x, xs[1] = xv.y;
        } else {
            xysum_grid(g.lane, s_c, cc, tt, xs);
            *reinterpret_cast<double2 *>(xs_row + i0) = make_double2(xs[0], xs[1]);
        }
        if (!pf_x_ok(s_c, valid, cc, tt, xs))
            bad = true;
        if (c + 1 < g.n_blocks && !same_bits(read_lane(xs[1], 63), rec[1].s_in))
            bad = true;
        float m_;
        const float est[kR] = {fit_value_known(Sv.x, xs[0], fk, m_), fit_value_known(Sv.y, xs[1], fk, m_)};
        const float est_before = c ? fit_value_known(S_front, s_c, fk, m_) : st.phaseEstimate;
        const float est_prev0 = wave_up1(est[1], est_before);
        const float2 rw = *reinterpret_cast<const float2 *>(raw_row + i0);
        const int2 k = *reinterpret_cast<const int2 *>(k_row + i0);
        const bool sure0 = __builtin_fabsf(est_prev0 - y.x) < 3.0f && __builtin_fabsf(y.x) < 65536.0f;
        const bool sure1 = __builtin_fabsf(est[0] - y.y) < 3.0f && __builtin_fabsf(y.y) < 65536.0f;
        if (!vote_all((sure0 || !valid[0]) && (sure1 || !valid[1]))) {
            const long long w0 = unwrap_count(est_prev0, (double)rw.x, c), w1 = unwrap_count(est[0], (double)rw.y, c);
            if ((valid[0] && w0 != (long long)k.x) || (valid[1] && w1 != (long long)k.y)) {
                bad_k = true;
                if (round == 0 && w0 == (long long)(int)w0 && w1 == (long long)(int)w1)
                    *reinterpret_cast<int2 *>(sc.k + g.off + i0) = make_int2((int)w0, (int)w1);
            }
        }
        *reinterpret_cast<float2 *>(est_row + i0) = make_float2(est[0], est[1]);
    }
    if (vote_any(bad) && g.lane == 0)
        atomicOr(&sc.chan[bi].fail, kPfFailXySum);
    if (vote_any(bad_k) && g.lane == 0)
        atomicOr(&sc.chan[bi].fail, kPfFailUnwrap);
}

__global__ __launch_bounds__(64) void pf_retry_kernel(const ChanPlan *__restrict__ plans, const uint32_t *__restrict__ list, PfScratch sc)
{
    const uint32_t bi = list[blockIdx.x];
    if (!pf_mine(plans[bi]) || (threadIdx.x & 63) != 0)
        return;
    const uint32_t f = sc.chan[bi].fail;
    if (f & kPfFailUnwrap)
        *sc.hint = 1u;
    const bool again = f == kPfFailUnwrap;
    sc.chan[bi].retry = again ? 1u : 0u;
    if (again)
        sc.chan[bi].fail = 0u;
}

}
#endif
```

### psk_soft_amd/csrc/psk_plan.h

```cpp
#ifndef PSK_PLAN_H
#define PSK_PLAN_H

#include <stdint.h>

#define PSK_PKT_ID_cs16 1
#define PSK_PKT_ID_cs8 3
#define PSK_PKT_ID_cf16 4

namespace psk {

enum PlanMode : uint32_t {
    PLAN_SKIP = 0,
    PLAN_FAST = 1,
    PLAN_SEQ = 2,
    PLAN_SEQ_S1 = 3,
};

enum LfFlags : uint32_t {
    LF_RECOMPUTE = 1u,
    PLAN_QPSK_SIGN_MAP = 2u,
    PLAN_TILED = 4u,
    PLAN_PFIT = 8u,
    PLAN_ANYFRONT = 16u,
    PLAN_NO_WRAP = 32u,
    PLAN_CARRY_DRIFT = 64u,
    PLAN_TIES_HANDOVER = 128u,
    PLAN_CS16 = 256u,
    PLAN_CS16_IN_PLACE = 512u,
    PLAN_CS8 = 1024u,
    PLAN_CS8_IN_PLACE = 2048u,
    PLAN_CF16 = 4096u,
    PLAN_CF16_IN_PLACE = 8192u,
    PLAN_FARFIT = 16384u,
};


constexpr uint32_t kResyncCount = 1048576u;

struct CvtDesc {
    const uint32_t *src;
    float *dst;
    uint64_t n;
};

constexpr bool ering_dynamic(int S) { return S == 9 || S == 10; }

struct ChanPlan {
    const float *in;
    float *soft;
    int16_t *bits;
    float *phase;
    int16_t *sidx;
    uint64_t n_in;
    uint64_t n_out;
    uint32_t mode;
    uint32_t S;
    uint32_t A;
    uint32_t M;
    uint32_t bpb;
    uint32_t diff;
    uint32_t ring_len0;
    uint32_t ring_len1;
    uint32_t ring_src;
    uint32_t lf_flags;
    uint32_t lf_n;
    uint32_t lf_head;
    uint32_t lf_len0;
    uint32_t lf_count0;
    uint32_t count0;
    float lf_xdelta;
    uint32_t tile_blocks;
    uint32_t tile_base;
    uint32_t far_row;
    uint64_t tile_off;
    uint32_t *handed_over;
};

constexpr unsigned kPlanHeaderBytes = 128u;
#if defined(__HIPCC__) || defined(__CUDACC__)
__host__ __device__
#endif
inline uint32_t *plan_header(const ChanPlan *plans)
{
    return reinterpret_cast<uint32_t *>(const_cast<char *>(reinterpret_cast<const char *>(plans)) - kPlanHeaderBytes);
}

struct TileInfo {
    uint32_t umax, umin1;
    uint32_t refuse;
    float gap_rel;
    float wmax;
    uint32_t stat_exact;
    uint32_t last_k;
    float cap;
    float last0_re, last0_im;
    float emax;
    uint32_t pad2;
};

struct PfTile {
    int jsum;
    int pad;
    double dsum;
    double dlast;
    double xsum;
};
struct PfBlock {
    double bsum;
    double a, b;
    double kmul;
    double D0s, D1s;
    int flags;
    int pad;
};
struct PfWalk {
    double s_in;
    int slow;
    int pad;
};
struct PfChan {
    uint32_t fail, done, slow_blocks;
    uint32_t retry;
    double ySum_c, xySum_c;
};
struct PfScratch {
    int *k;
    float *y;
    double *S;
    double *c;
    float *tt;
    double *xs;
    PfTile *tile;
    PfBlock *blk;
    PfWalk *walk;
    PfChan *chan;
    uint32_t *hint;
};

struct ChanState {
    double lf_ySum;
    double lf_xySum;
    float last_re;
    float last_im;
    float phaseEstimate;
    float lf_den;
    float lf_xavg;
    float lf_m;
    float lf_b;
    uint32_t guard;
    uint32_t stat_blocks;
    uint32_t stat_extra;
    uint32_t last_k;
    uint32_t stat_exact;
    uint32_t stat_chain;
    float emax_hint;
    uint32_t pad_state;
    uint32_t stat_pfit;
};

}
#endif
```

### psk_soft_amd/csrc/psk_tile.hip

```cpp
#include "psk_tile_kernel.h"
#include "psk_pfit.h"
#include "psk_tile_any.h"

namespace psk {

constexpr int kAnyPhases = 16;
template <int NP>
__global__ __launch_bounds__(64) void psk_tile_front_any_kernel(const ChanPlan *__restrict__ plans, const uint32_t *__restrict__ list, uint32_t ch0,
                                                                const ChanState *__restrict__ states, const float2 *__restrict__ rings,
                                                                uint32_t ring_cap, TileInfo *__restrict__ tiles, float *__restrict__ t_raw,
                                                                float2 *__restrict__ t_s, PfChan *__restrict__ pf_chan)
{
    const int lane = threadIdx.x & 63;
    const uint32_t bi = list[blockIdx.y];
    const ChanPlan &p = plans[bi];
    if (!tile_plan_mine(p) || !(p.lf_flags & PLAN_ANYFRONT))
        return;
    const int n_out = (int)p.n_out;
    const int n_blocks = (n_out + kB - 1) / kB;
    const int c_begin = (int)(blockIdx.x * p.tile_blocks);
    if (c_begin >= n_blocks)
        return;
    if (blockIdx.x == 0 && lane == 0)
        pf_chan[bi].fail = pf_chan[bi].done = pf_chan[bi].slow_blocks = pf_chan[bi].retry = 0u;
    const int c_end = c_begin + (int)p.tile_blocks < n_blocks ? c_begin + (int)p.tile_blocks : n_blocks;
    const int i_begin = c_begin * kB, i_end = c_end * kB < n_out ? c_end * kB : n_out;
    const uint32_t ch = ch0 + bi;
    XView X;
    X.ring = reinterpret_cast<const f2g *>(rings + ((size_t)ch * 2u + p.ring_src) * ring_cap);
    X.in = reinterpret_cast<const f2g *>(p.in);
    X.L0 = p.ring_len0;
    const int S = (int)p.S, A = (int)p.A;
    const uint32_t M = p.M;
    const int nk = NP == 1 ? 1 : (S + kWave - 1) / kWave;
    const bool timing = S > 1;
    const AtanTabDev atab = atan_tab_dev(lane);
    float *raw_row = t_raw + p.tile_off;
    float2 *s_row = t_s + p.tile_off;

    double W[NP];
#pragma unroll
    for (int j = 0; j < NP; j++) W[j] = 0.0;
    unsigned umax = 0u, umin1 = 0xFFFFFFFFu;
    bool refuse = false;
    float emax = 0.0f;
    auto energy_at = [&](uint64_t j) -> float {
        const float2 v = x_at(X, j);
        const float e = norm_f(v.x, v.y);
        const unsigned eb = __float_as_uint(e);
        if (eb >= 0x7F800000u)
            refuse = true;
        umax = eb > umax ? eb : umax;
        umin1 = (eb - 1u) < umin1 ? (eb - 1u) : umin1;
        emax = __builtin_fmaxf(emax, e);
        return e;
    };
    auto energy = [&](long long tau, int k) -> float {
        return k < S ? energy_at((uint64_t)tau * (uint64_t)S + (uint64_t)k) : 0.0f;
    };
    constexpr int UW = NP == 1 ? 8 : NP == 4 ? 4 : 1;
    const long long tau_end = (long long)i_begin + A - 1;
    __shared__ float e_lds[kWave * 8], e_lds_out[kWave * 8];
    const bool staged = NP == 1 && timing;
    if (staged) {
        const uint64_t j1 = (uint64_t)tau_end * (uint64_t)S;
        const uint32_t per = (uint32_t)((kWave * 8) / S) * (uint32_t)S;
        for (uint64_t jb = (uint64_t)i_begin * (uint64_t)S; jb < j1; jb += per) {
            const uint32_t len = j1 - jb < per ? (uint32_t)(j1 - jb) : per;
#pragma unroll
            for (int r = 0; r < 8; r++) {
                const uint32_t o = (uint32_t)(lane + kWave * r);
                e_lds[o] = o < len ? energy_at(jb + o) : 0.0f;
            }
            wave_lds_fence();
            if (lane < S) {
                const int ns = (int)(len / (uint32_t)S);
                for (int t = 0; t < ns; t++) W[0] += (double)e_lds[t * S + lane];
            }
            wave_lds_fence();
        }
    }
    for (long long tau = i_begin; timing && !staged && tau < tau_end; tau += UW) {
        float e[UW][NP];
#pragma unroll
        for (int u = 0; u < UW; u++)
#pragma unroll
            for (int j = 0; j < NP; j++)
                e[u][j] = (tau + u < tau_end && j < nk) ? energy(tau + u, lane + kWave * j) : 0.0f;
#pragma unroll
        for (int u = 0; u < UW; u++)
#pragma unroll
            for (int j = 0; j < NP; j++)
                if (tau + u < tau_end && j < nk)
                    W[j] += (double)e[u][j];
    }
    float gap_rel = __builtin_inff(), wmax = 0.0f;
    int kb = 0, k_last = 0;
    constexpr int U = NP == 1 ? 8 : 1;
    for (int i0 = i_begin; i0 < i_end; i0 += U) {
        float e_in[U][NP], e_out[U][NP];
        if constexpr (U > 1) {
            if (timing) {
                const int nu = i_end - i0 < U ? i_end - i0 : U;
                const uint32_t len = (uint32_t)(nu * S);
                const uint64_t j_in = (uint64_t)((long long)i0 + A - 1) * (uint64_t)S, j_out = (uint64_t)i0 * (uint64_t)S;
#pragma unroll
                for (int r = 0; r < 8; r++) {
                    if ((uint32_t)(kWave * r) >= len)
                        break;
                    const uint32_t o = (uint32_t)(lane + kWave * r);
                    float ei = 0.0f, eo = 0.0f;
                    if (o < len) {
                        ei = energy_at(j_in + o);
                        const float2 v = x_at(X, j_out + o);
                        eo = norm_f(v.x, v.y);
                    }
                    e_lds[o] = ei;
                    e_lds_out[o] = eo;
                }
                wave_lds_fence();
#pragma unroll
                for (int u = 0; u < U; u++) {
                    const bool on = u < nu && lane < S;
                    e_in[u][0] = on ? e_lds[u * S + lane] : 0.0f;
                    e_out[u][0] = on ? e_lds_out[u * S + lane] : 0.0f;
                }
                wave_lds_fence();
            }
        }
        if constexpr (NP == 1) {
            if (timing) {
                double best[U], second[U];
                unsigned k_win[U];
#pragma unroll
                for (int u = 0; u < U; u++) {
                    W[0] += (double)e_in[u][0];
                    best[u] = lane < S ? W[0] : -__builtin_inf();
                    W[0] -= (double)e_out[u][0];
                    second[u] = best[u];
                }
                any_max_f64_multi(best);
#pragma unroll
                for (int u = 0; u < U; u++) k_win[u] = second[u] == best[u] ? (unsigned)lane : 0xFFFFFFFFu;
                any_min_u32_multi(k_win);
#pragma unroll
                for (int u = 0; u < U; u++) second[u] = (unsigned)lane == k_win[u] ? -__builtin_inf() : second[u];
                any_max_f64_multi(second);
#pragma unroll
                for (int u = 0; u < U; u++) {
                    const int i = i0 + u;
                    const bool live = i < i_end;
                    const int kbest = k_win[u] < (unsigned)S ? (int)k_win[u] : 0;
                    k_last = live ? kbest : k_last;
                    wmax = live ? __builtin_fmaxf(wmax, (float)best[u] * 1.0000002f) : wmax;
                    const float g = (float)(best[u] - second[u]) / (2.0f * drift_bound(i + 1 + kB, (uint32_t)A));
                    const float gap_new = (g < gap_rel) ? g : ((g == g) ? gap_rel : 0.0f);
                    gap_rel = live ? gap_new : gap_rel;
                    kb = (live && lane == (i & (kWave - 1))) ? kbest : kb;
                }
            }
        } else if (timing) {
#pragma unroll
            for (int u = 0; u < U; u++) {
                const int i = i0 + u;
                const bool live = U == 1 || i < i_end;
#pragma unroll
                for (int j = 0; j < NP; j++)
                    if (j < nk)
                        W[j] += (double)(U > 1 ? e_in[u][j] : energy((long long)i + A - 1, lane + kWave * j));
                AnyTop top;
                top.best = -__builtin_inf();
                top.second = -__builtin_inf();
                top.k = 0x7fffffff;
#pragma unroll
                for (int j = 0; j < NP; j++) {
                    const int k = lane + kWave * j;
                    if (j < nk && k < S) {
                        AnyTop one;
                        one.best = W[j];
                        one.second = -__builtin_inf();
                        one.k = k;
                        top = any_merge(top, one);
                    }
                }
                const double best = any_max_f64(top.best);
                const unsigned k_win = any_min_u32(top.best == best ? (unsigned)top.k : 0xFFFFFFFFu);
                const double second = any_max_f64((unsigned)top.k == k_win ? top.second : top.best);
                const int kbest = k_win < (unsigned)S ? (int)k_win : 0;
                k_last = live ? kbest : k_last;
                const float best_f = (float)best;
                wmax = live ? __builtin_fmaxf(wmax, best_f * 1.0000002f) : wmax;
                const float g = (float)(best - second) / (2.0f * drift_bound(i + 1 + kB, (uint32_t)A));
                const float gap_new = (g < gap_rel) ? g : ((g == g) ? gap_rel : 0.0f);
                gap_rel = live ? gap_new : gap_rel;
#pragma unroll
                for (int j = 0; j < NP; j++)
                    if (j < nk)
                        W[j] -= (double)(U > 1 ? e_out[u][j] : energy(i, lane + kWave * j));
                kb = (live && lane == (i & (kWave - 1))) ? kbest : kb;
            }
        }
        const int i = (i0 + U < i_end ? i0 + U : i_end) - 1;
        const int slot = i & (kWave - 1);
        if (slot == kWave - 1 || i == i_end - 1) {
            const int mine = i - slot + lane;
            const bool have = lane <= slot;
            const uint64_t j_pick = !have ? (uint64_t)X.L0 : timing ? (uint64_t)mine * (uint64_t)S + (uint64_t)kb : (uint64_t)X.L0 + (uint64_t)mine;
            const float2 pk = x_at(X, j_pick);
            cf32 sv;
            sv.re = pk.x, sv.im = pk.y;
            const cf32 pw = cpow_uint<false>(sv, M);
            const float raw = atan2f_wave(pw.im, pw.re, atab);
            if (have) {
                if (!(is_fin(pw.re) && is_fin(pw.im)))
                    refuse = true;
                raw_row[mine] = raw;
                s_row[mine] = pk;
                if (p.sidx && timing)
                    p.sidx[mine] = (int16_t)(unsigned short)kb;
            }
        }
    }
    const unsigned umax_w = wave_max_u32(umax), umin1_w = wave_min_u32(umin1);
    const bool refuse_w = vote_any(refuse);
    const float emax_w = wave_max_f32(__builtin_fmaxf(emax, 0.0f));
    if (lane == 0) {
        TileInfo &t = tiles[p.tile_base + blockIdx.x];
        t.umax = umax_w;
        t.umin1 = umin1_w;
        t.refuse = refuse_w ? 1u : 0u;
        t.gap_rel = gap_rel;
        t.wmax = wmax;
        t.stat_exact = (uint32_t)(c_end - c_begin);
        t.last_k = (uint32_t)k_last;
        t.cap = __builtin_inff();
        t.emax = emax_w;
    }
}

PSK_DEV void pf_commit(const ChanPlan &p, uint32_t bi, uint32_t ch, ChanState *st, float2 *rings, uint32_t ring_cap, float *yvs, uint32_t fit_cap,
                       float *yring, uint32_t ymask, TileInfo *ti, int n_tiles, int exact_blocks, const float2 *t_s, const float *t_est,
                       const PfScratch &sc, int lane)
{
    const int n_out = (int)p.n_out;
    const int n_blocks = (n_out + kB - 1) / kB;
    float2 *ring_base = rings + (size_t)ch * 2u * ring_cap;
    const float2 *ring_src = ring_base + (size_t)p.ring_src * ring_cap;
    float2 *ring_dst = ring_base + (size_t)(p.ring_src ^ 1u) * ring_cap;
    float *yv = yvs + (size_t)ch * fit_cap;
    XView X;
    X.ring = reinterpret_cast<const f2g *>(ring_src);
    X.in = reinterpret_cast<const f2g *>(p.in);
    X.L0 = p.ring_len0;

    const int n = (int)p.lf_n;
    const float *y_row = sc.y + p.tile_off;
    const uint32_t q_end = p.lf_len0 + (uint32_t)n_out;
    for (int j = lane; j < n; j += kWave) {
        const int t = n_out - n + j;
        yring[(q_end - (uint32_t)n + (uint32_t)j) & ymask] = t >= 0 ? y_row[t] : yv[(p.lf_head + (uint32_t)(t + n)) % fit_cap];
    }
    wave_lds_fence();
    FastCarry cy;
    cy.ySum = sc.S[p.tile_off + (uint64_t)(n_out - 1)];
    cy.xySum = sc.xs[p.tile_off + (uint64_t)(n_out - 1)];
    cy.est = t_est[p.tile_off + (uint64_t)(n_out - 1)];
    cy.last_re = st->last_re;
    cy.last_im = st->last_im;
    const float last0_re = cy.last_re, last0_im = cy.last_im;
    cy.den = st->lf_den;
    cy.xavg = st->lf_xavg;
    fit_denominator(p.lf_xdelta, p.lf_n, cy.den, cy.xavg);
    {
        const FitKnown fk = fit_known(p.lf_xdelta, p.lf_n, cy.den, cy.xavg);
        float m_hint;
        (void)fit_value_known(cy.ySum, cy.xySum, fk, m_hint);
        m_hint *= p.lf_xdelta;
        cy.slope = is_fin(m_hint) ? m_hint : 0.0f;
    }
    cy.m = cy.b = 0.0f;
    cy.wmax = __builtin_inff();
    cy.q = q_end;
    cy.last_k = ti[n_tiles - 1].last_k;
    cy.stat_blocks = (uint32_t)n_blocks;
    cy.stat_extra = 0;
    cy.stat_exact_blocks = (uint32_t)exact_blocks;
    cy.stat_chain = sc.chan[bi].slow_blocks;
    if (p.diff) {
        const float2 l = t_s[p.tile_off + (uint64_t)(n_out - 1)];
        cy.last_re = l.x;
        cy.last_im = l.y;
    }
    if (lane == 0) {
        ti[0].last0_re = last0_re;
        ti[0].last0_im = last0_im;
        sc.chan[bi].done = 1u;
    }
    call_epilogue(p, st, yv, fit_cap, yring, ymask, X, ring_dst, lane, cy, kGuardTiled);
    if (lane == 0)
        st->stat_pfit = 1u | (sc.chan[bi].retry ? 0x100u : 0u);
}

__global__ __launch_bounds__(64) void psk_tile_fit_kernel(const ChanPlan *__restrict__ plans, const uint32_t *__restrict__ list, uint32_t ch0,
                                                          ChanState *__restrict__ states, float2 *__restrict__ rings, uint32_t ring_cap,
                                                          float *__restrict__ yvs, uint32_t fit_cap, uint32_t y_len,
                                                          TileInfo *__restrict__ tiles, const float *__restrict__ t_raw,
                                                          const float2 *__restrict__ t_s, float *__restrict__ t_est, PfScratch sc)
{
    extern __shared__ __attribute__((aligned(16))) float lds_dyn[];
    float *const yring = lds_dyn;
    const uint32_t ymask = y_len - 1u;
    const int lane = threadIdx.x & 63;
    const uint32_t bi = list[blockIdx.x];
    const ChanPlan &p = plans[bi];
    if (!tile_plan_mine(p))
        return;
    const uint32_t ch = ch0 + bi;
    ChanState *st = &states[ch];
    const int n_out = (int)p.n_out;
    const int n_blocks = (n_out + kB - 1) / kB;
    const int n_tiles = (n_blocks + (int)p.tile_blocks - 1) / (int)p.tile_blocks;
    TileInfo *const ti = tiles + p.tile_base;

    int exact_blocks = 0;
    float emax = 0.0f;
    const bool refuse = tile_fold(p, ti, n_tiles, lane, exact_blocks, emax);
    if (lane == 0)
        st->emax_hint = emax;
    if (refuse) {
        if (lane == 0) {
            st->guard = 1u;
            atomicAdd(p.handed_over, 1u);
        }
        return;
    }
    if ((p.lf_flags & PLAN_PFIT) && sc.chan[bi].fail == 0u) {
        pf_commit(p, bi, ch, st, rings, ring_cap, yvs, fit_cap, yring, ymask, ti, n_tiles, exact_blocks, t_s, t_est, sc, lane);
        return;
    }

    float2 *ring_base = rings + (size_t)ch * 2u * ring_cap;
    const float2 *ring_src = ring_base + (size_t)p.ring_src * ring_cap;
    float2 *ring_dst = ring_base + (size_t)(p.ring_src ^ 1u) * ring_cap;
    float *yv = yvs + (size_t)ch * fit_cap;
    XView X;
    X.ring = reinterpret_cast<const f2g *>(ring_src);
    X.in = reinterpret_cast<const f2g *>(p.in);
    X.L0 = p.ring_len0;

    FastCarry cy;
    call_prologue(p, st, yv, fit_cap, yring, ymask, lane, cy);
    const float last0_re = cy.last_re, last0_im = cy.last_im;

    const uint32_t n = p.lf_n;
    const float xd = p.lf_xdelta;
    float den_s = cy.den, xavg_s = cy.xavg;
    if (n > 1)
        fit_denominator(xd, n, den_s, xavg_s);
    const FitKnown fk = fit_known(xd, n, den_s, xavg_s);
    const float *raw_row = t_raw + p.tile_off;
    float *est_row = t_est + p.tile_off;
    float2 nxt = *reinterpret_cast<const float2 *>(raw_row + 2 * lane);
    for (int c = 0; c < n_blocks; c++) {
        const int i0 = c * kB + 2 * lane;
        const float raw[kR] = {nxt.x, nxt.y};
        if (c + 1 < n_blocks)
            nxt = *reinterpret_cast<const float2 *>(raw_row + i0 + kB);
        const bool valid[kR] = {i0 < n_out, i0 + 1 < n_out};
        const int rem = n_out - c * kB;
        const int nvalid = rem < kB ? rem : kB;
        const int lane_last = (nvalid - 1) >> 1, r_last = (nvalid - 1) & 1;
        if (cy.chain_streak >> 16)
            __builtin_amdgcn_s_setprio(PSK_CHAIN_PRIO);
        else
            __builtin_amdgcn_s_setprio(0);
        float est[kR];
        fit_stage<false>(c, lane, n, xd, den_s, xavg_s, fk, valid, raw, nvalid, lane_last, r_last, yring, ymask, cy, est);
        if (__any(cy.refuse)) {
            if (lane == 0) {
                st->guard = 1u;
                atomicAdd(p.handed_over, 1u);
            }
            return;
        }
        *reinterpret_cast<float2 *>(est_row + i0) = make_float2(est[0], est[1]);
    }

    cy.last_k = ti[n_tiles - 1].last_k;
    cy.stat_exact_blocks = (uint32_t)exact_blocks;
    if (p.diff) {
        const float2 l = t_s[p.tile_off + (uint64_t)(n_out - 1)];
        cy.last_re = l.x;
        cy.last_im = l.y;
    }
    if (lane == 0) {
        ti[0].last0_re = last0_re;
        ti[0].last0_im = last0_im;
    }
    call_epilogue(p, st, yv, fit_cap, yring, ymask, X, ring_dst, lane, cy, kGuardTiled);
    if ((p.lf_flags & PLAN_PFIT) && lane == 0) {
        st->stat_pfit = sc.chan[bi].fail << 1;
        if (sc.chan[bi].fail & kPfFailUnwrap)
            *sc.hint = 1u;
    }
}

struct PipeCarry {
    FastCarry cy[kWave];
    unsigned umax, umin1, refuse, gap_b, cap_b, wmax_b;
    int exact_blocks;
    float emax;
    float last0_re, last0_im;
    uint32_t dead;
    uint32_t pad;
};
__global__ __launch_bounds__(64) void psk_tile_fit_range_kernel(const ChanPlan *__restrict__ plans, const uint32_t *__restrict__ list, uint32_t ch0,
                                                                ChanState *__restrict__ states, float2 *__restrict__ rings, uint32_t ring_cap,
                                                                float *__restrict__ yvs, uint32_t fit_cap, uint32_t y_len,
                                                                TileInfo *__restrict__ tiles, const float *__restrict__ t_raw,
                                                                const float2 *__restrict__ t_s, float *__restrict__ t_est,
                                                                PipeCarry *__restrict__ carry, float *__restrict__ carry_y, uint32_t tile0,
                                                                uint32_t ntiles)
{
    extern __shared__ __attribute__((aligned(16))) float lds_dyn[];
    float *const yring = lds_dyn;
    const uint32_t ymask = y_len - 1u;
    const int lane = threadIdx.x & 63;
    const uint32_t bi = list[blockIdx.x];
    const ChanPlan &p = plans[bi];
    if (!tile_plan_mine(p))
        return;
    const uint32_t ch = ch0 + bi;
    ChanState *st = &states[ch];
    const int n_out = (int)p.n_out;
    const int n_blocks = (n_out + kB - 1) / kB;
    const int n_tiles = (n_blocks + (int)p.tile_blocks - 1) / (int)p.tile_blocks;
    if ((int)tile0 >= n_tiles)
        return;
    const int t_end = (int)(tile0 + ntiles) < n_tiles ? (int)(tile0 + ntiles) : n_tiles;
    const bool first = tile0 == 0u, last = t_end == n_tiles;
    TileInfo *const ti = tiles + p.tile_base;
    PipeCarry &pc = carry[blockIdx.x];
    float *const ysave = carry_y + (size_t)blockIdx.x * y_len;
    if (!first && pc.dead)
        return;

    float emax = first ? 0.0f : pc.emax;
    unsigned umax = first ? 0u : pc.umax, umin1 = first ? 0xFFFFFFFFu : pc.umin1, refuse_b = first ? 0u : pc.refuse;
    unsigned gap_b = first ? 0x7F800000u : pc.gap_b, cap_b = first ? 0x7F800000u : pc.cap_b, wmax_b = first ? 0u : pc.wmax_b;
    int exact_blocks = 0;
    for (int j = (int)tile0 + lane; j < t_end; j += kWave) {
        const TileInfo t = ti[j];
        umax = t.umax > umax ? t.umax : umax;
        umin1 = t.umin1 < umin1 ? t.umin1 : umin1;
        refuse_b |= t.refuse;
        const unsigned g = __float_as_uint(t.gap_rel), cp = __float_as_uint(t.cap), w = __float_as_uint(t.wmax);
        gap_b = g < gap_b ? g : gap_b;
        cap_b = cp < cap_b ? cp : cap_b;
        wmax_b = w > wmax_b ? w : wmax_b;
        exact_blocks += (int)t.stat_exact;
        emax = __builtin_fmaxf(emax, t.emax);
    }
    emax = wave_max_f32(__builtin_fmaxf(emax, 0.0f));
    umax = wave_max_u32(umax);
    umin1 = wave_min_u32(umin1);
    gap_b = wave_min_u32(gap_b);
    cap_b = wave_min_u32(cap_b);
    wmax_b = wave_max_u32(wmax_b);
    exact_blocks = __builtin_amdgcn_readlane(wave_scan_i32(exact_blocks), 63) + (first ? 0 : pc.exact_blocks);
    bool refuse = __any(refuse_b != 0u);
    {
        const float wmax = __uint_as_float(wmax_b);
        if (!(wmax <= __uint_as_float(cap_b)) && !(wmax < 1.0e-37f))
            refuse = true;
        const bool ambiguous = !(__uint_as_float(gap_b) > wmax);
        if (umin1 != 0xFFFFFFFFu && ambiguous) {
            int eh = (int)(umax >> 23), el = (int)((umin1 + 1u) >> 23);
            eh = eh < 1 ? 1 : eh;
            el = el < 1 ? 1 : el;
            const int terms_log2 = 32 - __builtin_clz((unsigned)(p.A + 2u * kB));
            if (24 + (eh - el) + terms_log2 > 52)
                refuse = true;
        }
    }
    auto hand_over = [&]() {
        if (lane == 0) {
            st->emax_hint = emax;
            st->guard = 1u;
            atomicAdd(p.handed_over, 1u);
            pc.dead = 1u;
        }
    };
    if (refuse) {
        hand_over();
        return;
    }

    float2 *ring_base = rings + (size_t)ch * 2u * ring_cap;
    const float2 *ring_src = ring_base + (size_t)p.ring_src * ring_cap;
    float2 *ring_dst = ring_base + (size_t)(p.ring_src ^ 1u) * ring_cap;
    float *yv = yvs + (size_t)ch * fit_cap;
    XView X;
    X.ring = reinterpret_cast<const f2g *>(ring_src);
    X.in = reinterpret_cast<const f2g *>(p.in);
    X.L0 = p.ring_len0;

    FastCarry cy;
    float last0_re, last0_im;
    if (first) {
        call_prologue(p, st, yv, fit_cap, yring, ymask, lane, cy);
        last0_re = cy.last_re, last0_im = cy.last_im;
        if (lane == 0) {
            ti[0].last0_re = last0_re;
            ti[0].last0_im = last0_im;
        }
    } else {
        cy = pc.cy[lane];
        last0_re = pc.last0_re, last0_im = pc.last0_im;
        for (uint32_t j = lane; j < y_len; j += kWave) yring[j] = ysave[j];
        wave_lds_fence();
    }

    const uint32_t n = p.lf_n;
    const float xd = p.lf_xdelta;
    float den_s = cy.den, xavg_s = cy.xavg;
    if (n > 1)
        fit_denominator(xd, n, den_s, xavg_s);
    const FitKnown fk = fit_known(xd, n, den_s, xavg_s);
    const float *raw_row = t_raw + p.tile_off;
    float *est_row = t_est + p.tile_off;
    const int c0 = (int)tile0 * (int)p.tile_blocks;
    const int c1 = last ? n_blocks : t_end * (int)p.tile_blocks;
    __builtin_amdgcn_s_setprio(3);
    float2 nxt = *reinterpret_cast<const float2 *>(raw_row + c0 * kB + 2 * lane);
    for (int c = c0; c < c1; c++) {
        const int i0 = c * kB + 2 * lane;
        const float raw[kR] = {nxt.x, nxt.y};
        if (c + 1 < c1)
            nxt = *reinterpret_cast<const float2 *>(raw_row + i0 + kB);
        const bool valid[kR] = {i0 < n_out, i0 + 1 < n_out};
        const int rem = n_out - c * kB;
        const int nvalid = rem < kB ? rem : kB;
        const int lane_last = (nvalid - 1) >> 1, r_last = (nvalid - 1) & 1;
        float est[kR];
        fit_stage<false>(c, lane, n, xd, den_s, xavg_s, fk, valid, raw, nvalid, lane_last, r_last, yring, ymask, cy, est);
        if (__any(cy.refuse)) {
            hand_over();
            return;
        }
        *reinterpret_cast<float2 *>(est_row + i0) = make_float2(est[0], est[1]);
    }

    if (!last) {
        pc.cy[lane] = cy;
        wave_lds_fence();
        for (uint32_t j = lane; j < y_len; j += kWave) ysave[j] = yring[j];
        if (lane == 0) {
            pc.umax = umax, pc.umin1 = umin1, pc.refuse = refuse_b ? 1u : 0u, pc.gap_b = gap_b, pc.cap_b = cap_b, pc.wmax_b = wmax_b;
            pc.exact_blocks = exact_blocks;
            pc.emax = emax;
            pc.last0_re = last0_re, pc.last0_im = last0_im;
            pc.dead = 0u;
        }
        return;
    }
    if (lane == 0)
        st->emax_hint = emax;
    cy.last_k = ti[n_tiles - 1].last_k;
    cy.stat_exact_blocks = (uint32_t)exact_blocks;
    if (p.diff) {
        const float2 l = t_s[p.tile_off + (uint64_t)(n_out - 1)];
        cy.last_re = l.x;
        cy.last_im = l.y;
    }
    call_epilogue(p, st, yv, fit_cap, yring, ymask, X, ring_dst, lane, cy, kGuardTiled);
}

hipError_t launch_tile_fit_range(const ChanPlan *plans, const uint32_t *list, uint32_t ch0, uint32_t nch, ChanState *states, float2 *rings,
                                 uint32_t ring_cap, float *yvs, uint32_t fit_cap, uint32_t y_len, TileInfo *tiles, const float *t_raw,
                                 const float2 *t_s, float *t_est, void *carry, float *carry_y, uint32_t tile0, uint32_t ntiles,
                                 hipStream_t stream)
{
    if (!nch || !ntiles)
        return hipSuccess;
    hipLaunchKernelGGL(psk_tile_fit_range_kernel, dim3(nch), dim3(kWave), sizeof(float) * (size_t)y_len, stream, plans, list, ch0, states, rings,
                       ring_cap, yvs, fit_cap, y_len, tiles, t_raw, t_s, t_est, static_cast<PipeCarry *>(carry), carry_y, tile0, ntiles);
    return hipGetLastError();
}
size_t pipe_carry_bytes() { return sizeof(PipeCarry); }

__global__ __launch_bounds__(64) void pf_begin_kernel(const ChanPlan *__restrict__ plans, const uint32_t *__restrict__ list, uint32_t ch0,
                                                      const ChanState *__restrict__ states, const float *__restrict__ yvs, uint32_t fit_cap,
                                                      uint32_t y_len, PfScratch sc)
{
    extern __shared__ __attribute__((aligned(16))) float lds_dyn[];
    const int lane = threadIdx.x & 63;
    const uint32_t bi = list[blockIdx.x];
    const ChanPlan &p = plans[bi];
    if (!pf_mine(p))
        return;
    FastCarry cy;
    call_prologue(p, &states[ch0 + bi], yvs + (size_t)(ch0 + bi) * fit_cap, fit_cap, lds_dyn, y_len - 1u, lane, cy);
    if (lane == 0) {
        sc.chan[bi].ySum_c = cy.ySum;
        sc.chan[bi].xySum_c = cy.xySum;
    }
}

__global__ __launch_bounds__(64) void psk_tile_back_kernel(const ChanPlan *__restrict__ plans, const uint32_t *__restrict__ list, uint32_t ch0,
                                                           const ChanState *__restrict__ states, const TileInfo *__restrict__ tiles,
                                                           const float2 *__restrict__ t_s, const float *__restrict__ t_est,
                                                           uint32_t tile0, uint32_t early)
{
    const int lane = threadIdx.x & 63;
    const uint32_t bi = list[blockIdx.y];
    const ChanPlan &p = plans[bi];
    if (!tile_plan_mine(p) || (!early && states[ch0 + bi].guard != kGuardTiled))
        return;
    const int n_out = (int)p.n_out;
    const int n_blocks = (n_out + kB - 1) / kB;
    const int c_begin = (int)((blockIdx.x + tile0) * p.tile_blocks);
    if (c_begin >= n_blocks)
        return;
    const int c_end = c_begin + (int)p.tile_blocks < n_blocks ? c_begin + (int)p.tile_blocks : n_blocks;
    const uint32_t M = p.M;
    const bool m_pow2 = M != 0 && (M & (M - 1)) == 0;
    const float inv_M = uni(1.0f / (float)(M ? M : 1));
    const AtanTabDev atab = atan_tab_dev(lane);
    const bool qpsk_sign_map = (p.lf_flags & PLAN_QPSK_SIGN_MAP) != 0;
    const float2 *s_row = t_s + p.tile_off;
    const float *est_row = t_est + p.tile_off;
    for (int c = c_begin; c < c_end; c++) {
        const int i0 = c * kB + 2 * lane;
        const bool valid[kR] = {i0 < n_out, i0 + 1 < n_out};
        const float4 sv = *reinterpret_cast<const float4 *>(s_row + i0);
        const float2 ev = *reinterpret_cast<const float2 *>(est_row + i0);
        cf32 s[kR];
        s[0].re = sv.x, s[0].im = sv.y, s[1].re = sv.z, s[1].im = sv.w;
        const float est[kR] = {ev.x, ev.y};
        cf32 last_c;
        last_c.re = last_c.im = 0.0f;
        if (p.diff) {
            if (c == 0) {
                last_c.re = tiles[p.tile_base].last0_re;
                last_c.im = tiles[p.tile_base].last0_im;
            } else {
                const float2 l = s_row[c * kB - 1];
                last_c.re = l.x, last_c.im = l.y;
            }
        }
        output_stage<true, true>(p, c, i0, valid, s, est, last_c, atab, qpsk_sign_map, m_pow2, inv_M);
    }
}

#define PSK_TDECL(S) hipError_t launch_tile_front_S##S##_H1(PSK_TILE_FRONT_ARGS);
PSK_TDECL(2) PSK_TDECL(3) PSK_TDECL(4) PSK_TDECL(5) PSK_TDECL(6) PSK_TDECL(7) PSK_TDECL(8) PSK_TDECL(9)
PSK_TDECL(10) PSK_TDECL(11) PSK_TDECL(12) PSK_TDECL(13) PSK_TDECL(14) PSK_TDECL(15) PSK_TDECL(16)

bool tile_front_has(int S, int H) { return H == 1 && S >= 2 && S <= 16; }

hipError_t launch_tile_front(int S, int H, PSK_TILE_FRONT_ARGS)
{
#define PSK_TCASE(Sv)       \
    if (S == Sv && H == 1) \
        return launch_tile_front_S##Sv##_H1(plans, list, ch0, nch, max_tiles, states, rings, ring_cap, r_len, tiles, t_raw, t_s, pf_chan, tile0, stream);
    PSK_TCASE(2) PSK_TCASE(3) PSK_TCASE(4) PSK_TCASE(5) PSK_TCASE(6) PSK_TCASE(7) PSK_TCASE(8) PSK_TCASE(9)
    PSK_TCASE(10) PSK_TCASE(11) PSK_TCASE(12) PSK_TCASE(13) PSK_TCASE(14) PSK_TCASE(15) PSK_TCASE(16)
    return hipErrorInvalidValue;
}

hipError_t launch_tile_front_any(const ChanPlan *plans, const uint32_t *list, uint32_t ch0, uint32_t nch, uint32_t max_tiles, uint32_t max_S,
                                 const ChanState *states, const float2 *rings, uint32_t ring_cap, TileInfo *tiles, float *t_raw, float2 *t_s,
                                 PfChan *pf_chan, hipStream_t stream)
{
    if (!nch || !max_tiles)
        return hipSuccess;
    for (uint32_t off = 0; off < nch; off += kGridYMax) {
        const uint32_t n = nch - off < kGridYMax ? nch - off : kGridYMax;
        if (max_S <= 64u)
            hipLaunchKernelGGL(psk_tile_front_any_kernel<1>, dim3(max_tiles, n), dim3(kWave), 0, stream, plans, list + off, ch0, states, rings,
                               ring_cap, tiles, t_raw, t_s, pf_chan);
        else if (max_S <= 256u)
            hipLaunchKernelGGL(psk_tile_front_any_kernel<4>, dim3(max_tiles, n), dim3(kWave), 0, stream, plans, list + off, ch0, states, rings,
                               ring_cap, tiles, t_raw, t_s, pf_chan);
        else
            hipLaunchKernelGGL(psk_tile_front_any_kernel<kAnyPhases>, dim3(max_tiles, n), dim3(kWave), 0, stream, plans, list + off, ch0, states,
                               rings, ring_cap, tiles, t_raw, t_s, pf_chan);
    }
    return hipGetLastError();
}

hipError_t launch_tile_fit(const ChanPlan *plans, const uint32_t *list, uint32_t ch0, uint32_t nch, ChanState *states, float2 *rings,
                           uint32_t ring_cap, float *yvs, uint32_t fit_cap, uint32_t y_len, TileInfo *tiles, const float *t_raw,
                           const float2 *t_s, float *t_est, const PfScratch &sc, hipStream_t stream)
{
    if (!nch)
        return hipSuccess;
    static LdsGrant granted;
    if (const hipError_t e = lds_grant(reinterpret_cast<const void *>(&psk_tile_fit_kernel), sizeof(float) * (size_t)y_len, granted))
        return e;
    hipLaunchKernelGGL(psk_tile_fit_kernel, dim3(nch), dim3(kWave), sizeof(float) * (size_t)y_len, stream, plans, list, ch0, states, rings,
                       ring_cap, yvs, fit_cap, y_len, tiles, t_raw, t_s, t_est, sc);
    return hipGetLastError();
}

hipError_t launch_pfit(const ChanPlan *plans, const uint32_t *list, uint32_t ch0, uint32_t nch, uint32_t max_tiles, ChanState *states,
                       float2 *rings, uint32_t ring_cap, float *yvs, uint32_t fit_cap, uint32_t y_len, TileInfo *tiles, const float *t_raw,
                       const float2 *t_s, float *t_est, const PfScratch &sc, bool second_round, hipStream_t stream)
{
    if (!nch || !max_tiles)
        return hipSuccess;
    const dim3 wave(kWave);
    static LdsGrant granted_b;
    if (const hipError_t e = lds_grant(reinterpret_cast<const void *>(&pf_begin_kernel), sizeof(float) * (size_t)y_len, granted_b))
        return e;
    for (uint32_t off = 0; off < nch; off += kGridYMax) {
        const uint32_t n = nch - off < kGridYMax ? nch - off : kGridYMax;
        const uint32_t *const l = list + off;
        const dim3 grid(max_tiles, n);
        hipLaunchKernelGGL(pf_begin_kernel, dim3(n), wave, sizeof(float) * (size_t)y_len, stream, plans, l, ch0, states, yvs, fit_cap, y_len, sc);
        hipLaunchKernelGGL(pf_unwrap_kernel, grid, wave, 0, stream, plans, l, ch0, states, t_raw, sc);
        for (int round = 0; round <= (second_round ? 1 : 0); round++) {
            if (round)
                hipLaunchKernelGGL(pf_retry_kernel, dim3(n), wave, 0, stream, plans, l, sc);
            hipLaunchKernelGGL(pf_y_kernel, grid, wave, 0, stream, plans, l, ch0, states, t_raw, sc, round);
            hipLaunchKernelGGL(pf_ydiff_kernel, grid, wave, 0, stream, plans, l, ch0, yvs, fit_cap, sc, round);
            hipLaunchKernelGGL(pf_ysum_kernel, grid, wave, 0, stream, plans, l, ch0, states, yvs, fit_cap, sc, round);
            hipLaunchKernelGGL(pf_xblock_kernel, grid, wave, 0, stream, plans, l, ch0, states, sc, round);
            hipLaunchKernelGGL(pf_xwalk_kernel, dim3(n), wave, 0, stream, plans, l, sc.blk, sc, round);
            hipLaunchKernelGGL(pf_verify_kernel, grid, wave, 0, stream, plans, l, ch0, states, yvs, fit_cap, t_raw, t_est, sc, round);
        }
    }
    return hipGetLastError();
}

hipError_t launch_tile_back(const ChanPlan *plans, const uint32_t *list, uint32_t ch0, uint32_t nch, uint32_t max_tiles,
                            const ChanState *states, const TileInfo *tiles, const float2 *t_s, const float *t_est, uint32_t tile0,
                            uint32_t early, hipStream_t stream)
{
    if (!nch || !max_tiles)
        return hipSuccess;
    for (uint32_t off = 0; off < nch; off += kGridYMax) {
        const uint32_t n = nch - off < kGridYMax ? nch - off : kGridYMax;
        hipLaunchKernelGGL(psk_tile_back_kernel, dim3(max_tiles, n), dim3(kWave), 0, stream, plans, list + off, ch0, states, tiles, t_s, t_est, tile0, early);
    }
    return hipGetLastError();
}

}
```

Measured before the change: 459,000.

## Fuse parallel-fit stages and recompute prefix sums instead of storing scratch arrays

Merges the prologue kernel into the unwrap kernel as an extra block column and folds the y-generation kernel into the ydiff kernel. It also drops the per-sample S, c and tt double scratch arrays, so later stages recompute the y prefix sums and xy operands from y and tile offsets. End-of-channel carries are now stored per channel rather than read back from the full arrays. This is meant to cut HBM traffic and kernel launches in the parallel-fit path, in exchange for redundant wave scans and extra bookkeeping records.

```diff
diff --git a/psk_soft_amd/csrc/psk_capi.cpp b/psk_soft_amd/csrc/psk_capi.cpp
--- a/psk_soft_amd/csrc/psk_capi.cpp
+++ b/psk_soft_amd/csrc/psk_capi.cpp
@@ -926,8 +926,8 @@
     psk::PfScratch &pf = h->pf;
     bool got = false;
     PSK_HIP(grow_scratch({scratch_buf(&h->d_tiles, cnt), scratch_buf(&h->d_traw, syms), scratch_buf(&h->d_test, syms), scratch_buf(&h->d_ts, syms),
-                          scratch_buf(&pf.k, psyms), scratch_buf(&pf.y, psyms), scratch_buf(&pf.S, psyms), scratch_buf(&pf.c, psyms),
-                          scratch_buf(&pf.tt, psyms), scratch_buf(&pf.xs, psyms), scratch_buf(&pf.tile, pcnt),
+                          scratch_buf(&pf.kr, psyms), scratch_buf(&pf.k, psyms), scratch_buf(&pf.y, psyms), scratch_buf(&pf.xs, psyms),
+                          scratch_buf(&pf.tile, pcnt),
                           scratch_buf(&pf.blk, psyms / 128u + 1u), scratch_buf(&pf.walk, psyms / 128u + 1u)},
                          &got));
     if (got && !pf.chan) {
@@ -1747,7 +1747,7 @@
         if (h->d_traw) (void)hipFree(h->d_traw);
         if (h->d_test) (void)hipFree(h->d_test);
         if (h->d_ts) (void)hipFree(h->d_ts);
-        for (void *q : {(void *)h->pf.k, (void *)h->pf.y, (void *)h->pf.S, (void *)h->pf.c, (void *)h->pf.tt, (void *)h->pf.xs,
+        for (void *q : {(void *)h->pf.kr, (void *)h->pf.k, (void *)h->pf.y, (void *)h->pf.xs,
                         (void *)h->pf.tile, (void *)h->pf.blk, (void *)h->pf.walk, (void *)h->pf.chan})
             if (q) (void)hipFree(q);
         if (h->pf.hint) (void)hipHostFree(h->pf.hint);
diff --git a/psk_soft_amd/csrc/psk_pfit.h b/psk_soft_amd/csrc/psk_pfit.h
--- a/psk_soft_amd/csrc/psk_pfit.h
+++ b/psk_soft_amd/csrc/psk_pfit.h
@@ -35,17 +35,74 @@
     return t >= n ? y_row[t - n] : yv[(p.lf_head + (uint32_t)t) % fit_cap];
 }
 
+PSK_DEV float pf_yval(float raw, int k, double two_pi) { return (float)((double)raw + (double)(long long)k * two_pi); }
+PSK_DEV double pf_soff(const PfScratch &sc, uint32_t bi, const PfGeo &g, int tile)
+{
+    double s = 0.0;
+    for (int j = g.lane; j < tile; j += kWave) s += sc.tile[g.tbase + j].dsum;
+    return sc.chan[bi].ySum_c + wave_sum_f64(s);
+}
+struct PfYSum {
+    double a0, a1, S0, S1;
+    double total;
+};
+PSK_DEV PfYSum pf_ysum_block(double soff, double run, float2 y, float z0, float z1, bool v0, bool v1)
+{
+    const double d0 = v0 ? (double)y.x - (double)z0 : 0.0;
+    const double d1 = v1 ? (double)y.y - (double)z1 : 0.0;
+    const double incl = wave_scan_f64(d0 + d1);
+    PfYSum o;
+    o.a0 = (run + wave_up1(incl, 0.0)) + d0;
+    o.a1 = o.a0 + d1;
+    o.S0 = soff + o.a0;
+    o.S1 = soff + o.a1;
+    o.total = read_lane(incl, 63);
+    return o;
+}
+PSK_DEV double pf_block_last(int n_out, int c, double v0, double v1)
+{
+    const int rem = n_out - c * kB;
+    const int last = (rem < kB ? rem : kB) - 1;
+    return read_lane((last & 1) ? v1 : v0, last >> 1);
+}
+PSK_DEV void pf_xy_operands(float xd, float sizef, double S_before, const PfYSum &ys, float2 y, float z0f, float z1f, bool v0, bool v1,
+                            double (&a)[kR], double (&cc)[kR], double (&tt)[kR])
+{
+    const double z0 = v0 ? (double)z0f : 0.0, z1 = v1 ? (double)z1f : 0.0;
+    const double Sp = wave_up1(ys.S1, S_before);
+    a[0] = Sp - z0, a[1] = ys.S0 - z1;
+    float t0 = y.x * sizef;
+    t0 = t0 * xd;
+    float t1 = y.y * sizef;
+    t1 = t1 * xd;
+    cc[0] = v0 ? (double)xd * a[0] : 0.0, cc[1] = v1 ? (double)xd * a[1] : 0.0;
+    tt[0] = v0 ? (double)t0 : 0.0, tt[1] = v1 ? (double)t1 : 0.0;
+}
+
 constexpr float kPfSteep = 0.12f;
 __global__ __launch_bounds__(64) void pf_unwrap_kernel(const ChanPlan *__restrict__ plans, const uint32_t *__restrict__ list, uint32_t ch0,
-                                                       const ChanState *__restrict__ states, const float *__restrict__ t_raw, PfScratch sc)
-{
+                                                       const ChanState *__restrict__ states, const float *__restrict__ yvs, uint32_t fit_cap,
+                                                       uint32_t y_len, const float *__restrict__ t_raw, PfScratch sc)
+{
+    extern __shared__ __attribute__((aligned(16))) float lds_dyn[];
     const uint32_t bi = list[blockIdx.y];
     const ChanPlan &p = plans[bi];
+    if (!pf_mine(p))
+        return;
+    if (blockIdx.x + 1u == gridDim.x) {
+        FastCarry cy;
+        call_prologue(p, &states[ch0 + bi], yvs + (size_t)(ch0 + bi) * fit_cap, fit_cap, lds_dyn, y_len - 1u, (int)(threadIdx.x & 63), cy);
+        if ((threadIdx.x & 63) == 0) {
+            sc.chan[bi].ySum_c = cy.ySum;
+            sc.chan[bi].xySum_c = cy.xySum;
+        }
+        return;
+    }
     PfGeo g;
-    if (!pf_mine(p) || !pf_geo(p, g))
+    if (!pf_geo(p, g))
         return;
     const float *raw_row = t_raw + g.off;
-    int *k_row = sc.k + g.off;
+    int *k_row = sc.kr + g.off;
     const float inv2pi = 0.15915494f, two_pi = 6.2831853f;
     const ChanState &st = states[ch0 + bi];
     const bool steep = !(__builtin_fabsf(st.lf_m) < kPfSteep);
@@ -104,8 +161,25 @@
         sc.tile[g.tbase + g.tile].jsum = run;
 }
 
-__global__ __launch_bounds__(64) void pf_y_kernel(const ChanPlan *__restrict__ plans, const uint32_t *__restrict__ list, uint32_t ch0,
-                                                  const ChanState *__restrict__ states, const float *__restrict__ t_raw, PfScratch sc, int round)
+struct PfZSrc {
+    float r;
+    int k;
+};
+PSK_DEV PfZSrc pf_zsrc(const ChanPlan &p, const float *raw_row, const int *kin_row, const float *yv, uint32_t fit_cap, int u)
+{
+    PfZSrc o;
+    if (u < 0) {
+        o.r = yv[(p.lf_head + (uint32_t)(u + (int)p.lf_n)) % fit_cap];
+        o.k = 0;
+    } else {
+        o.r = raw_row[u];
+        o.k = kin_row[u];
+    }
+    return o;
+}
+__global__ __launch_bounds__(64) void pf_ydiff_kernel(const ChanPlan *__restrict__ plans, const uint32_t *__restrict__ list, uint32_t ch0,
+                                                      const ChanState *__restrict__ states, const float *__restrict__ yvs, uint32_t fit_cap,
+                                                      const float *__restrict__ t_raw, PfScratch sc, int round)
 {
     const uint32_t bi = list[blockIdx.y];
     const ChanPlan &p = plans[bi];
@@ -113,37 +187,72 @@
     if (!pf_in_round(p, sc, bi, round) || !pf_geo(p, g))
         return;
     const float *raw_row = t_raw + g.off;
+    const int *kin_row = (round == 0 ? sc.kr : sc.k) + g.off;
     int *k_row = sc.k + g.off;
     float *y_row = sc.y + g.off;
-    int koff = 0;
+    const float *yv = yvs + (size_t)(ch0 + bi) * fit_cap;
+    const int n = (int)p.lf_n;
+    const int tile_len = (int)p.tile_blocks * kB;
+    const int u_begin = g.c_begin * kB - n;
+    const int jA = u_begin > 0 ? u_begin / tile_len : 0;
+    const int u_split = (jA + 1) * tile_len;
+    int koff = 0, koffA = 0, koffB = 0;
     if (round == 0) {
-        for (int j = g.lane; j < g.tile; j += kWave) koff += sc.tile[g.tbase + j].jsum;
+        for (int j = g.lane; j < g.tile; j += kWave) {
+            const int js = sc.tile[g.tbase + j].jsum;
+            koff += js;
+            koffA += j < jA ? js : 0;
+            koffB += j <= jA ? js : 0;
+        }
         koff = __builtin_amdgcn_readlane(wave_scan_i32(koff), 63);
-        if (!(__builtin_fabsf(states[ch0 + bi].lf_m) < kPfSteep))
-            koff += (int)unwrap_count(states[ch0 + bi].phaseEstimate, (double)raw_row[0]);
-    }
-    float2 rw_n = *reinterpret_cast<const float2 *>(raw_row + g.c_begin * kB + 2 * g.lane);
-    int2 k_n = *reinterpret_cast<const int2 *>(k_row + g.c_begin * kB + 2 * g.lane);
+        koffA = __builtin_amdgcn_readlane(wave_scan_i32(koffA), 63);
+        koffB = __builtin_amdgcn_readlane(wave_scan_i32(koffB), 63);
+        if (!(__builtin_fabsf(states[ch0 + bi].lf_m) < kPfSteep)) {
+            const int first = (int)unwrap_count(states[ch0 + bi].phaseEstimate, (double)raw_row[0]);
+            koff += first;
+            koffA += first;
+            koffB += first;
+        }
+    }
+    double run = 0.0, dlast = 0.0;
+    const int j0 = g.c_begin * kB + 2 * g.lane;
+    float2 rw_n = *reinterpret_cast<const float2 *>(raw_row + j0);
+    int2 k_n = *reinterpret_cast<const int2 *>(kin_row + j0);
+    PfZSrc z0_n = pf_zsrc(p, raw_row, kin_row, yv, fit_cap, j0 - n), z1_n = pf_zsrc(p, raw_row, kin_row, yv, fit_cap, j0 + 1 - n);
     for (int c = g.c_begin; c < g.c_end; c++) {
         const int i0 = c * kB + 2 * g.lane;
         const float2 rw = rw_n;
         int2 k = k_n;
+        const PfZSrc zs0 = z0_n, zs1 = z1_n;
         if (c + 1 < g.c_end) {
             rw_n = *reinterpret_cast<const float2 *>(raw_row + i0 + kB);
-            k_n = *reinterpret_cast<const int2 *>(k_row + i0 + kB);
+            k_n = *reinterpret_cast<const int2 *>(kin_row + i0 + kB);
+            z0_n = pf_zsrc(p, raw_row, kin_row, yv, fit_cap, i0 + kB - n);
+            z1_n = pf_zsrc(p, raw_row, kin_row, yv, fit_cap, i0 + kB + 1 - n);
         }
         k.x += koff;
         k.y += koff;
-        *reinterpret_cast<int2 *>(k_row + i0) = k;
+        if (round == 0)
+            *reinterpret_cast<int2 *>(k_row + i0) = k;
         const double two_pi = PSK_KD(kTwoPi, c);
-        const float y0 = (float)((double)rw.x + (double)(long long)k.x * two_pi);
-        const float y1 = (float)((double)rw.y + (double)(long long)k.y * two_pi);
-        *reinterpret_cast<float2 *>(y_row + i0) = make_float2(y0, y1);
-    }
-}
-
-__global__ __launch_bounds__(64) void pf_ydiff_kernel(const ChanPlan *__restrict__ plans, const uint32_t *__restrict__ list, uint32_t ch0,
-                                                      const float *__restrict__ yvs, uint32_t fit_cap, PfScratch sc, int round)
+        const float2 y = make_float2(pf_yval(rw.x, k.x, two_pi), pf_yval(rw.y, k.y, two_pi));
+        *reinterpret_cast<float2 *>(y_row + i0) = y;
+        const int u0 = i0 - n, u1 = u0 + 1;
+        const float z0 = u0 < 0 ? zs0.r : pf_yval(zs0.r, zs0.k + (u0 < u_split ? koffA : koffB), two_pi);
+        const float z1 = u1 < 0 ? zs1.r : pf_yval(zs1.r, zs1.k + (u1 < u_split ? koffA : koffB), two_pi);
+        const PfYSum ys = pf_ysum_block(0.0, run, y, z0, z1, i0 < g.n_out, i0 + 1 < g.n_out);
+        run += ys.total;
+        dlast = pf_block_last(g.n_out, c, ys.a0, ys.a1);
+    }
+    if (g.lane == 0) {
+        sc.tile[g.tbase + g.tile].dsum = run;
+        sc.tile[g.tbase + g.tile].dlast = dlast;
+    }
+}
+
+__global__ __launch_bounds__(64) void pf_ysum_kernel(const ChanPlan *__restrict__ plans, const uint32_t *__restrict__ list, uint32_t ch0,
+                                                     const ChanState *__restrict__ states, const float *__restrict__ yvs, uint32_t fit_cap,
+                                                     PfScratch sc, int round)
 {
     const uint32_t bi = list[blockIdx.y];
     const ChanPlan &p = plans[bi];
@@ -152,104 +261,48 @@
         return;
     const float *y_row = sc.y + g.off;
     const float *yv = yvs + (size_t)(ch0 + bi) * fit_cap;
-    double *S_row = sc.S + g.off;
-    double run = 0.0, dlast = 0.0;
+    const double soff = pf_soff(sc, bi, g, g.tile);
+    bool bad = false;
+    if (g.tile > 0) {
+        const double soff_b = pf_soff(sc, bi, g, g.tile - 1);
+        bad = !same_bits(soff_b + sc.tile[g.tbase + g.tile - 1].dlast, soff);
+    }
+    const float xd = p.lf_xdelta;
+    const float sizef = (float)(p.lf_n - 1u);
+    double S_before = soff;
+    double run = 0.0, xrun = 0.0;
     const int j0 = g.c_begin * kB + 2 * g.lane;
     float2 y_n = *reinterpret_cast<const float2 *>(y_row + j0);
     float z0_n = pf_z(p, y_row, yv, fit_cap, j0), z1_n = pf_z(p, y_row, yv, fit_cap, j0 + 1);
     for (int c = g.c_begin; c < g.c_end; c++) {
         const int i0 = c * kB + 2 * g.lane;
+        const bool v0 = i0 < g.n_out, v1 = i0 + 1 < g.n_out;
         const float2 y = y_n;
-        const float z0 = z0_n, z1 = z1_n;
+        const float z0f = z0_n, z1f = z1_n;
         if (c + 1 < g.c_end) {
             y_n = *reinterpret_cast<const float2 *>(y_row + i0 + kB);
             z0_n = pf_z(p, y_row, yv, fit_cap, i0 + kB);
             z1_n = pf_z(p, y_row, yv, fit_cap, i0 + kB + 1);
         }
-        const bool v0 = i0 < g.n_out, v1 = i0 + 1 < g.n_out;
-        const double d0 = v0 ? (double)y.x - (double)z0 : 0.0;
-        const double d1 = v1 ? (double)y.y - (double)z1 : 0.0;
-        const double incl = wave_scan_f64(d0 + d1);
-        const double a0 = (run + wave_up1(incl, 0.0)) + d0;
-        *reinterpret_cast<double2 *>(S_row + i0) = make_double2(a0, a0 + d1);
-        run += read_lane(incl, 63);
-        const int rem = g.n_out - c * kB;
-        const int last = (rem < kB ? rem : kB) - 1;
-        dlast = read_lane((last & 1) ? a0 + d1 : a0, last >> 1);
+        const PfYSum ys = pf_ysum_block(soff, run, y, z0f, z1f, v0, v1);
+        double a[kR], cc[kR], tt[kR];
+        pf_xy_operands(xd, sizef, S_before, ys, y, z0f, z1f, v0, v1, a, cc, tt);
+        bad = bad || (v0 && !same_bits(a[0] + (double)y.x, ys.S0)) || (v1 && !same_bits(a[1] + (double)y.y, ys.S1));
+        const double bs = wave_sum_f64((tt[0] - cc[0]) + (tt[1] - cc[1]));
+        if (g.lane == 0) {
+            PfBlock &rec = sc.blk[g.bbase + c];
+            rec.bsum = bs;
+            rec.yrun = run;
+            rec.ybefore = S_before;
+        }
+        xrun += bs;
+        run += ys.total;
+        S_before = pf_block_last(g.n_out, c, ys.S0, ys.S1);
     }
     if (g.lane == 0) {
-        sc.tile[g.tbase + g.tile].dsum = run;
-        sc.tile[g.tbase + g.tile].dlast = dlast;
-    }
-}
-
-__global__ __launch_bounds__(64) void pf_ysum_kernel(const ChanPlan *__restrict__ plans, const uint32_t *__restrict__ list, uint32_t ch0,
-                                                     const ChanState *__restrict__ states, const float *__restrict__ yvs, uint32_t fit_cap,
-                                                     PfScratch sc, int round)
-{
-    const uint32_t bi = list[blockIdx.y];
-    const ChanPlan &p = plans[bi];
-    PfGeo g;
-    if (!pf_in_round(p, sc, bi, round) || !pf_geo(p, g))
-        return;
-    const float *y_row = sc.y + g.off;
-    const float *yv = yvs + (size_t)(ch0 + bi) * fit_cap;
-    double *S_row = sc.S + g.off;
-    double *c_row = sc.c + g.off;
-    float *t_row = sc.tt + g.off;
-    double soff = 0.0;
-    for (int j = g.lane; j < g.tile; j += kWave) soff += sc.tile[g.tbase + j].dsum;
-    soff = sc.chan[bi].ySum_c + wave_sum_f64(soff);
-    bool bad = false;
-    if (g.tile > 0) {
-        double soff_b = 0.0;
-        for (int j = g.lane; j < g.tile - 1; j += kWave) soff_b += sc.tile[g.tbase + j].dsum;
-        soff_b = sc.chan[bi].ySum_c + wave_sum_f64(soff_b);
-        bad = !same_bits(soff_b + sc.tile[g.tbase + g.tile - 1].dlast, soff);
-    }
-    const float xd = p.lf_xdelta;
-    const float sizef = (float)(p.lf_n - 1u);
-    double S_before = soff;
-    double xrun = 0.0;
-    const int j0 = g.c_begin * kB + 2 * g.lane;
-    float2 y_n = *reinterpret_cast<const float2 *>(y_row + j0);
-    double2 dl_n = *reinterpret_cast<const double2 *>(S_row + j0);
-    float z0_n = pf_z(p, y_row, yv, fit_cap, j0), z1_n = pf_z(p, y_row, yv, fit_cap, j0 + 1);
-    for (int c = g.c_begin; c < g.c_end; c++) {
-        const int i0 = c * kB + 2 * g.lane;
-        const bool v0 = i0 < g.n_out, v1 = i0 + 1 < g.n_out;
-        const float2 y = y_n;
-        const double2 dl = dl_n;
-        const float z0f = z0_n, z1f = z1_n;
-        if (c + 1 < g.c_end) {
-            y_n = *reinterpret_cast<const float2 *>(y_row + i0 + kB);
-            dl_n = *reinterpret_cast<const double2 *>(S_row + i0 + kB);
-            z0_n = pf_z(p, y_row, yv, fit_cap, i0 + kB);
-            z1_n = pf_z(p, y_row, yv, fit_cap, i0 + kB + 1);
-        }
-        const double S0 = soff + dl.x, S1 = soff + dl.y;
-        const double z0 = v0 ? (double)z0f : 0.0, z1 = v1 ? (double)z1f : 0.0;
-        const double Sp = wave_up1(S1, S_before);
-        const double a0 = Sp - z0, a1 = S0 - z1;
-        bad = bad || (v0 && !same_bits(a0 + (double)y.x, S0)) || (v1 && !same_bits(a1 + (double)y.y, S1));
-        const double c0 = (double)xd * a0, c1 = (double)xd * a1;
-        float t0 = y.x * sizef;
-        t0 = t0 * xd;
-        float t1 = y.y * sizef;
-        t1 = t1 * xd;
-        *reinterpret_cast<double2 *>(S_row + i0) = make_double2(S0, S1);
-        *reinterpret_cast<double2 *>(c_row + i0) = make_double2(c0, c1);
-        *reinterpret_cast<float2 *>(t_row + i0) = make_float2(t0, t1);
-        const double bs = wave_sum_f64((v0 ? (double)t0 - c0 : 0.0) + (v1 ? (double)t1 - c1 : 0.0));
-        if (g.lane == 0)
-            sc.blk[g.bbase + c].bsum = bs;
-        xrun += bs;
-        const int rem = g.n_out - c * kB;
-        const int last = (rem < kB ? rem : kB) - 1;
-        S_before = read_lane((last & 1) ? S1 : S0, last >> 1);
-    }
-    if (g.lane == 0)
         sc.tile[g.tbase + g.tile].xsum = xrun;
+        sc.tile[g.tbase + g.tile].soff = soff;
+    }
     if (vote_any(bad) && g.lane == 0)
         atomicOr(&sc.chan[bi].fail, kPfFailYSum);
 }
@@ -304,32 +357,42 @@
 }
 
 __global__ __launch_bounds__(64) void pf_xblock_kernel(const ChanPlan *__restrict__ plans, const uint32_t *__restrict__ list, uint32_t ch0,
-                                                       const ChanState *__restrict__ states, PfScratch sc, int round)
+                                                       const ChanState *__restrict__ states, const float *__restrict__ yvs, uint32_t fit_cap,
+                                                       PfScratch sc, int round)
 {
     const uint32_t bi = list[blockIdx.y];
     const ChanPlan &p = plans[bi];
     PfGeo g;
     if (!pf_in_round(p, sc, bi, round) || !pf_geo(p, g))
         return;
-    const double *c_row = sc.c + g.off;
-    const float *t_row = sc.tt + g.off;
+    const float *y_row = sc.y + g.off;
+    const float *yv = yvs + (size_t)(ch0 + bi) * fit_cap;
+    const float xd = p.lf_xdelta;
+    const float sizef = (float)(p.lf_n - 1u);
     double s_pred = 0.0;
     for (int j = g.lane; j < g.tile; j += kWave) s_pred += sc.tile[g.tbase + j].xsum;
     s_pred = sc.chan[bi].xySum_c + wave_sum_f64(s_pred);
     int prev_scale = -1;
     if (g.c_begin > 0) {
-        const double s_before = s_pred - sc.blk[g.bbase + g.c_begin - 1].bsum;
-        const int eb_b = (__double2hiint(s_before - c_row[(g.c_begin - 1) * kB]) >> 20) & 0x7ff;
+        const PfBlock &pb = sc.blk[g.bbase + g.c_begin - 1];
+        const double s_before = s_pred - pb.bsum;
+        const double c_first_b = (double)xd * (pb.ybefore - (double)pf_z(p, y_row, yv, fit_cap, (g.c_begin - 1) * kB));
+        const int eb_b = (__double2hiint(s_before - c_first_b) >> 20) & 0x7ff;
         if (eb_b >= 60 && eb_b <= 2040)
             prev_scale = 2 * eb_b + (!(__builtin_fabs(s_before) < pow2_biased(eb_b + 1)) ? 1 : 0);
     }
+    const double soff = sc.tile[g.tbase + g.tile].soff;
+    double S_before = soff, run = 0.0;
     for (int c = g.c_begin; c < g.c_end; c++) {
         const int i0 = c * kB + 2 * g.lane;
         const bool v0 = i0 < g.n_out, v1 = i0 + 1 < g.n_out;
-        const double2 cv = *reinterpret_cast<const double2 *>(c_row + i0);
-        const float2 tv = *reinterpret_cast<const float2 *>(t_row + i0);
-        const double cc[kR] = {v0 ? cv.x : 0.0, v1 ? cv.y : 0.0};
-        const double tt[kR] = {v0 ? (double)tv.x : 0.0, v1 ? (double)tv.y : 0.0};
+        const float2 y = *reinterpret_cast<const float2 *>(y_row + i0);
+        const float z0f = pf_z(p, y_row, yv, fit_cap, i0), z1f = pf_z(p, y_row, yv, fit_cap, i0 + 1);
+        const PfYSum ys = pf_ysum_block(soff, run, y, z0f, z1f, v0, v1);
+        double a_[kR], cc[kR], tt[kR];
+        pf_xy_operands(xd, sizef, S_before, ys, y, z0f, z1f, v0, v1, a_, cc, tt);
+        run += ys.total;
+        S_before = pf_block_last(g.n_out, c, ys.S0, ys.S1);
         const double c_first = read_lane(cc[0], 0);
         const double r_first = s_pred - c_first;
         const int eb = (__double2hiint(r_first) >> 20) & 0x7ff;
@@ -338,7 +401,7 @@
         rec.a = __builtin_inf();
         rec.b = -__builtin_inf();
         rec.kmul = rec.D0s = rec.D1s = 0.0;
-        rec.flags = rec.pad = 0;
+        rec.flags = 0;
         int scale_id = -1;
         if (eb >= 60 && eb <= 2040) {
             const double inv_q = pow2_biased(2098 - eb);
@@ -390,8 +453,11 @@
             }
         }
         prev_scale = scale_id;
-        if (g.lane == 0)
-            sc.blk[g.bbase + c] = rec;
+        if (g.lane == 0) {
+            PfBlock &out = sc.blk[g.bbase + c];
+            out.a = rec.a, out.b = rec.b, out.kmul = rec.kmul, out.D0s = rec.D0s, out.D1s = rec.D1s;
+            out.flags = rec.flags;
+        }
         s_pred += rec.bsum;
     }
 }
@@ -404,30 +470,39 @@
 }
 
 struct PfOps {
-    double2 cv;
-    float2 tv;
+    float2 y;
+    float z0, z1;
+    double soff, run, S_before;
 };
-PSK_DEV PfOps pf_load_ops(int lane, int b, const double *c_row, const float *t_row)
+PSK_DEV PfOps pf_load_ops(int lane, int b, const ChanPlan &p, const float *y_row, const float *yv, uint32_t fit_cap, const PfBlock *blk,
+                          const PfTile *tile)
 {
     const int i0 = b * kB + 2 * lane;
     PfOps o;
-    o.cv = *reinterpret_cast<const double2 *>(c_row + i0);
-    o.tv = *reinterpret_cast<const float2 *>(t_row + i0);
+    o.y = *reinterpret_cast<const float2 *>(y_row + i0);
+    o.z0 = pf_z(p, y_row, yv, fit_cap, i0);
+    o.z1 = pf_z(p, y_row, yv, fit_cap, i0 + 1);
+    o.soff = tile[(uint32_t)b / p.tile_blocks].soff;
+    o.run = blk[b].yrun;
+    o.S_before = blk[b].ybefore;
     return o;
 }
-PSK_DEV double pf_walk_block(int lane, int b, int n_out, double s_c, const PfOps &ops, double *xs_row, bool try_grid, bool &grid_failed)
+PSK_DEV double pf_walk_block(int lane, int b, int n_out, double s_c, float xd, float sizef, const PfOps &ops, double *xs_row, bool try_grid,
+                             bool &grid_failed)
 {
     const int i0 = b * kB + 2 * lane;
     const bool valid[kR] = {i0 < n_out, i0 + 1 < n_out};
+    double cc[kR], tt[kR];
 #ifdef PSK_DIAG_WALK_NOLOAD
-    const double2 cv = make_double2(s_c * 0.25, s_c * 0.125);
-    const float2 tv = make_float2((float)lane, 1.0f);
+    cc[0] = valid[0] ? s_c * 0.25 : 0.0, cc[1] = valid[1] ? s_c * 0.125 : 0.0;
+    tt[0] = valid[0] ? (double)(float)lane : 0.0, tt[1] = valid[1] ? 1.0 : 0.0;
 #else
-    const double2 cv = ops.cv;
-    const float2 tv = ops.tv;
+    {
+        const PfYSum ys = pf_ysum_block(ops.soff, ops.run, ops.y, ops.z0, ops.z1, valid[0], valid[1]);
+        double a_[kR];
+        pf_xy_operands(xd, sizef, ops.S_before, ys, ops.y, ops.z0, ops.z1, valid[0], valid[1], a_, cc, tt);
+    }
 #endif
-    const double cc[kR] = {valid[0] ? cv.x : 0.0, valid[1] ? cv.y : 0.0};
-    const double tt[kR] = {valid[0] ? (double)tv.x : 0.0, valid[1] ? (double)tv.y : 0.0};
     double xs[kR];
     bool done = false;
 #ifdef PSK_DIAG_WALK_NOCHAIN
@@ -464,8 +539,9 @@
     const int lo = bperm_addr(src << 2, __double2loint(v)), hi = bperm_addr(src << 2, __double2hiint(v));
     return __hiloint2double(hi, lo);
 }
-__global__ __launch_bounds__(64) void pf_xwalk_kernel(const ChanPlan *__restrict__ plans, const uint32_t *__restrict__ list,
-                                                      const PfBlock *__restrict__ blk_all, PfScratch sc, int round)
+__global__ __launch_bounds__(64) void pf_xwalk_kernel(const ChanPlan *__restrict__ plans, const uint32_t *__restrict__ list, uint32_t ch0,
+                                                      const float *__restrict__ yvs, uint32_t fit_cap, const PfBlock *__restrict__ blk_all,
+                                                      PfScratch sc, int round)
 {
     const uint32_t bi = list[blockIdx.x];
     const ChanPlan &p = plans[bi];
@@ -476,8 +552,11 @@
     const int n_blocks = (n_out + kB - 1) / kB;
     const PfBlock *const blk = blk_all + (uint32_t)(p.tile_off / kB);
     PfWalk *const walk = sc.walk + (uint32_t)(p.tile_off / kB);
-    const double *c_row = sc.c + p.tile_off;
-    const float *t_row = sc.tt + p.tile_off;
+    const PfTile *const tile = sc.tile + p.tile_base;
+    const float *y_row = sc.y + p.tile_off;
+    const float *yv = yvs + (size_t)(ch0 + bi) * fit_cap;
+    const float xd = p.lf_xdelta;
+    const float sizef = (float)(p.lf_n - 1u);
     double *xs_row = sc.xs + p.tile_off;
     double s_c = sc.chan[bi].xySum_c;
     uint32_t slow_blocks = 0;
@@ -541,19 +620,19 @@
                 continue;
             }
             int fs = f;
-            PfOps ops = pf_load_ops(lane, b0 + fs, c_row, t_row);
+            PfOps ops = pf_load_ops(lane, b0 + fs, p, y_row, yv, fit_cap, blk, tile);
             bool grid_first = !(a_f < b_f);
             bool grid_failed = false;
             for (;;) {
                 const bool more = fs + 1 < nb;
                 PfOps ahead = ops;
                 if (more)
-                    ahead = pf_load_ops(lane, b0 + fs + 1, c_row, t_row);
+                    ahead = pf_load_ops(lane, b0 + fs + 1, p, y_row, yv, fit_cap, blk, tile);
                 if (lane == fs) {
                     s_in_mine = s_c;
                     slow_mine = 1;
                 }
-                s_c = pf_walk_block(lane, b0 + fs, n_out, s_c, ops, xs_row, grid_first, grid_failed);
+                s_c = pf_walk_block(lane, b0 + fs, n_out, s_c, xd, sizef, ops, xs_row, grid_first, grid_failed);
                 slow_blocks++;
                 start = fs + 1;
                 if (!more)
@@ -595,9 +674,8 @@
     const float *raw_row = t_raw + g.off;
     const int *k_row = sc.k + g.off;
     const float *y_row = sc.y + g.off;
-    const double *S_row = sc.S + g.off;
     const float *yv = yvs + (size_t)(ch0 + bi) * fit_cap;
-    double *xs_row = sc.xs + g.off;
+    const double *xs_row = sc.xs + g.off;
     float *est_row = t_est + g.off;
     const uint32_t n = p.lf_n;
     const float xd = p.lf_xdelta;
@@ -606,37 +684,32 @@
     fit_denominator(xd, n, den_s, xavg_s);
     const FitKnown fk = fit_known(xd, n, den_s, xavg_s);
     bool bad = false, bad_k = false;
+    double x_last = 0.0;
+    const double soff = sc.tile[g.tbase + g.tile].soff;
+    double S_front = soff, run = 0.0;
     for (int c = g.c_begin; c < g.c_end; c++) {
         const int i0 = c * kB + 2 * g.lane;
         const bool valid[kR] = {i0 < g.n_out, i0 + 1 < g.n_out};
         const PfWalk *rec = sc.walk + g.bbase + c;
         const double s_c = rec->s_in;
-        const double2 Sv = *reinterpret_cast<const double2 *>(S_row + i0);
         const float2 y = *reinterpret_cast<const float2 *>(y_row + i0);
-        const double S_front = c ? S_row[c * kB - 1] : sc.chan[bi].ySum_c + 0.0;
-        const double Sp = wave_up1(Sv.y, S_front);
-        const double z0 = valid[0] ? (double)pf_z(p, y_row, yv, fit_cap, i0) : 0.0, z1 = valid[1] ? (double)pf_z(p, y_row, yv, fit_cap, i0 + 1) : 0.0;
-        const double a0 = Sp - z0, a1 = Sv.x - z1;
-        float t0 = y.x * sizef;
-        t0 = t0 * xd;
-        float t1 = y.y * sizef;
-        t1 = t1 * xd;
-        const double cc[kR] = {valid[0] ? (double)xd * a0 : 0.0, valid[1] ? (double)xd * a1 : 0.0};
-        const double tt[kR] = {valid[0] ? (double)t0 : 0.0, valid[1] ? (double)t1 : 0.0};
+        const float z0f = pf_z(p, y_row, yv, fit_cap, i0), z1f = pf_z(p, y_row, yv, fit_cap, i0 + 1);
+        const PfYSum Sv = pf_ysum_block(soff, run, y, z0f, z1f, valid[0], valid[1]);
+        double a_[kR], cc[kR], tt[kR];
+        pf_xy_operands(xd, sizef, S_front, Sv, y, z0f, z1f, valid[0], valid[1], a_, cc, tt);
         double xs[kR];
         if (rec->slow) {
             const double2 xv = *reinterpret_cast<const double2 *>(xs_row + i0);
             xs[0] = xv.x, xs[1] = xv.y;
         } else {
             xysum_grid(g.lane, s_c, cc, tt, xs);
-            *reinterpret_cast<double2 *>(xs_row + i0) = make_double2(xs[0], xs[1]);
         }
         if (!pf_x_ok(s_c, valid, cc, tt, xs))
             bad = true;
         if (c + 1 < g.n_blocks && !same_bits(read_lane(xs[1], 63), rec[1].s_in))
             bad = true;
         float m_;
-        const float est[kR] = {fit_value_known(Sv.x, xs[0], fk, m_), fit_value_known(Sv.y, xs[1], fk, m_)};
+        const float est[kR] = {fit_value_known(Sv.S0, xs[0], fk, m_), fit_value_known(Sv.S1, xs[1], fk, m_)};
         const float est_before = c ? fit_value_known(S_front, s_c, fk, m_) : st.phaseEstimate;
         const float est_prev0 = wave_up1(est[1], est_before);
         const float2 rw = *reinterpret_cast<const float2 *>(raw_row + i0);
@@ -652,6 +725,13 @@
             }
         }
         *reinterpret_cast<float2 *>(est_row + i0) = make_float2(est[0], est[1]);
+        run += Sv.total;
+        S_front = pf_block_last(g.n_out, c, Sv.S0, Sv.S1);
+        x_last = pf_block_last(g.n_out, c, xs[0], xs[1]);
+    }
+    if (g.c_end == g.n_blocks && g.lane == 0) {
+        sc.chan[bi].ySum_end = S_front;
+        sc.chan[bi].xySum_end = x_last;
     }
     if (vote_any(bad) && g.lane == 0)
         atomicOr(&sc.chan[bi].fail, kPfFailXySum);
diff --git a/psk_soft_amd/csrc/psk_plan.h b/psk_soft_amd/csrc/psk_plan.h
--- a/psk_soft_amd/csrc/psk_plan.h
+++ b/psk_soft_amd/csrc/psk_plan.h
@@ -104,6 +104,7 @@
     double dsum;
     double dlast;
     double xsum;
+    double soff;
 };
 struct PfBlock {
     double bsum;
@@ -112,6 +113,8 @@
     double D0s, D1s;
     int flags;
     int pad;
+    double yrun;
+    double ybefore;
 };
 struct PfWalk {
     double s_in;
@@ -122,13 +125,12 @@
     uint32_t fail, done, slow_blocks;
     uint32_t retry;
     double ySum_c, xySum_c;
+    double ySum_end, xySum_end;
 };
 struct PfScratch {
+    int *kr;
     int *k;
     float *y;
-    double *S;
-    double *c;
-    float *tt;
     double *xs;
     PfTile *tile;
     PfBlock *blk;
diff --git a/psk_soft_amd/csrc/psk_tile.hip b/psk_soft_amd/csrc/psk_tile.hip
--- a/psk_soft_amd/csrc/psk_tile.hip
+++ b/psk_soft_amd/csrc/psk_tile.hip
@@ -262,8 +262,8 @@
     }
     wave_lds_fence();
     FastCarry cy;
-    cy.ySum = sc.S[p.tile_off + (uint64_t)(n_out - 1)];
-    cy.xySum = sc.xs[p.tile_off + (uint64_t)(n_out - 1)];
+    cy.ySum = sc.chan[bi].ySum_end;
+    cy.xySum = sc.chan[bi].xySum_end;
     cy.est = t_est[p.tile_off + (uint64_t)(n_out - 1)];
     cy.last_re = st->last_re;
     cy.last_im = st->last_im;
@@ -589,24 +589,6 @@
 }
 size_t pipe_carry_bytes() { return sizeof(PipeCarry); }
 
-__global__ __launch_bounds__(64) void pf_begin_kernel(const ChanPlan *__restrict__ plans, const uint32_t *__restrict__ list, uint32_t ch0,
-                                                      const ChanState *__restrict__ states, const float *__restrict__ yvs, uint32_t fit_cap,
-                                                      uint32_t y_len, PfScratch sc)
-{
-    extern __shared__ __attribute__((aligned(16))) float lds_dyn[];
-    const int lane = threadIdx.x & 63;
-    const uint32_t bi = list[blockIdx.x];
-    const ChanPlan &p = plans[bi];
-    if (!pf_mine(p))
-        return;
-    FastCarry cy;
-    call_prologue(p, &states[ch0 + bi], yvs + (size_t)(ch0 + bi) * fit_cap, fit_cap, lds_dyn, y_len - 1u, lane, cy);
-    if (lane == 0) {
-        sc.chan[bi].ySum_c = cy.ySum;
-        sc.chan[bi].xySum_c = cy.xySum;
-    }
-}
-
 __global__ __launch_bounds__(64) void psk_tile_back_kernel(const ChanPlan *__restrict__ plans, const uint32_t *__restrict__ list, uint32_t ch0,
                                                            const ChanState *__restrict__ states, const TileInfo *__restrict__ tiles,
                                                            const float2 *__restrict__ t_s, const float *__restrict__ t_est,
@@ -712,22 +694,21 @@
         return hipSuccess;
     const dim3 wave(kWave);
     static LdsGrant granted_b;
-    if (const hipError_t e = lds_grant(reinterpret_cast<const void *>(&pf_begin_kernel), sizeof(float) * (size_t)y_len, granted_b))
+    if (const hipError_t e = lds_grant(reinterpret_cast<const void *>(&pf_unwrap_kernel), sizeof(float) * (size_t)y_len, granted_b))
         return e;
     for (uint32_t off = 0; off < nch; off += kGridYMax) {
         const uint32_t n = nch - off < kGridYMax ? nch - off : kGridYMax;
         const uint32_t *const l = list + off;
         const dim3 grid(max_tiles, n);
-        hipLaunchKernelGGL(pf_begin_kernel, dim3(n), wave, sizeof(float) * (size_t)y_len, stream, plans, l, ch0, states, yvs, fit_cap, y_len, sc);
-        hipLaunchKernelGGL(pf_unwrap_kernel, grid, wave, 0, stream, plans, l, ch0, states, t_raw, sc);
+        hipLaunchKernelGGL(pf_unwrap_kernel, dim3(max_tiles + 1u, n), wave, sizeof(float) * (size_t)y_len, stream, plans, l, ch0, states, yvs,
+                           fit_cap, y_len, t_raw, sc);
         for (int round = 0; round <= (second_round ? 1 : 0); round++) {
             if (round)
                 hipLaunchKernelGGL(pf_retry_kernel, dim3(n), wave, 0, stream, plans, l, sc);
-            hipLaunchKernelGGL(pf_y_kernel, grid, wave, 0, stream, plans, l, ch0, states, t_raw, sc, round);
-            hipLaunchKernelGGL(pf_ydiff_kernel, grid, wave, 0, stream, plans, l, ch0, yvs, fit_cap, sc, round);
+            hipLaunchKernelGGL(pf_ydiff_kernel, grid, wave, 0, stream, plans, l, ch0, states, yvs, fit_cap, t_raw, sc, round);
             hipLaunchKernelGGL(pf_ysum_kernel, grid, wave, 0, stream, plans, l, ch0, states, yvs, fit_cap, sc, round);
-            hipLaunchKernelGGL(pf_xblock_kernel, grid, wave, 0, stream, plans, l, ch0, states, sc, round);
-            hipLaunchKernelGGL(pf_xwalk_kernel, dim3(n), wave, 0, stream, plans, l, sc.blk, sc, round);
+            hipLaunchKernelGGL(pf_xblock_kernel, grid, wave, 0, stream, plans, l, ch0, states, yvs, fit_cap, sc, round);
+            hipLaunchKernelGGL(pf_xwalk_kernel, dim3(n), wave, 0, stream, plans, l, ch0, yvs, fit_cap, sc.blk, sc, round);
             hipLaunchKernelGGL(pf_verify_kernel, grid, wave, 0, stream, plans, l, ch0, states, yvs, fit_cap, t_raw, t_est, sc, round);
         }
     }
```

New measurement: 456,200, median of 3. No clear change (-0.6%).
